# jhoobergs/Thesis-pbrt-v3

Hardware: AMD Instinct MI355X
Metric: Mrays/s (higher is better)
Workload: dtype f32; 1 GPU; Sponza-class atrium STAND-IN (311,728 tris, matte+plastic, point light; the reference ships no Sponza geometry) 700x700, halton 1024 spp, path maxdepth 5, bvh; spp_total=1024, tiles=16x16 round-robin over 1 GPU(s), parallelism=tile-dp1, film_merge=none (single GPU)

## Files before the change

thesis-pbrt-v3_amd/__init__.py:

```python
import ctypes as C
import os

import numpy as np

_HERE = os.path.dirname(os.path.abspath(__file__))
LIB_PATH = os.environ.get("HPRT_LIB") or os.path.join(_HERE, "lib", "libhprt.so")


class HprtError(RuntimeError):
    def __init__(self, code, msg):
        super().__init__("hprt error %d: %s" % (code, msg))
        self.code = code


E_INVALID, E_IO, E_PARSE, E_NO_DEVICE, E_DEVICE, E_UNSUPPORTED = -1, -2, -3, -4, -5, -6
RENDER_COUNT_WORK = 1
RENDER_PIXEL_STATS = 2
RENDER_COUNT_TRACED = 4
RENDER_TRACE_ALL = 8
RENDER_EXPORT_FOREIGN = 16
ACCEL_BVH, ACCEL_KDTREE, ACCEL_RBSP = 0, 1, 2
ACCEL_BSP = ACCEL_RBSP
KD_MAX_DEPTH = 64
RBSP_MAX_DEPTH = 64
# ... 181 lines not shown

class SceneDesc(C.Structure):
    _fields_ = [("nodes", C.c_void_p), ("n_nodes", C.c_uint32), ("prim_order", C.c_void_p), ("n_prims", C.c_uint32),
                ("shapes", C.POINTER(ShapeDesc)), ("n_shapes", C.c_uint32),
                ("materials", C.POINTER(MaterialDesc)), ("n_materials", C.c_uint32),
                ("lights", C.POINTER(LightDesc)), ("n_lights", C.c_uint32), ("light_strategy", C.c_int32),
                ("textures", C.c_void_p), ("n_textures", C.c_uint32),
                ("objects", C.c_void_p), ("n_objects", C.c_uint32), ("instances", C.c_void_p), ("n_instances", C.c_uint32),
                ("top", C.c_void_p), ("n_top", C.c_uint32)]


def _load():
    if not os.path.exists(LIB_PATH):
        raise ImportError("hprt: %s is missing — run `python thesis-pbrt-v3_amd/build.py` (hipcc, gfx950). "
                          "There is no CPU fallback." % LIB_PATH)
    lib = C.CDLL(LIB_PATH)
    vp, cp, i32, u32, u64, sz = C.c_void_p, C.c_char_p, C.c_int32, C.c_uint32, C.c_uint64, C.c_size_t
    P = C.POINTER
    sig = {
        "hprt_last_error": (cp, []),
        "hprt_version": (cp, []),
        "hprt_model_parse": (C.c_int, [cp, P(cp), C.c_int, P(vp)]),
        "hprt_model_load": (C.c_int, [cp, P(vp)]),
        "hprt_model_save": (C.c_int, [vp, cp]),
        "hprt_model_save_compact": (C.c_int, [vp, cp]),
        "hprt_model_destroy": (None, [vp]),
        "hprt_model_get_options": (C.c_int, [vp, P(RenderOptions)]),
        "hprt_model_set_options": (C.c_int, [vp, P(RenderOptions)]),
        "hprt_model_counts": (C.c_int, [vp, P(u64)]),
        "hprt_model_warnings": (cp, [vp]),
        "hprt_model_texture_info": (C.c_int, [vp, C.c_uint32, P(C.c_int32), P(C.c_float)]),
        "hprt_model_texture_level": (C.c_int, [vp, C.c_uint32, C.c_uint32, P(C.c_int32), vp]),
        "hprt_bvh_build": (C.c_int, [vp, P(vp)]),
        "hprt_bvh_build_from_bounds": (C.c_int, [sz, vp, vp, C.c_int, C.c_int, C.c_int, P(vp)]),
        "hprt_bvh_destroy": (None, [vp]),
        "hprt_bvh_info": (C.c_int, [vp, P(u32), P(C.c_float)]),
        "hprt_bvh_copy": (C.c_int, [vp, vp, vp]),
        "hprt_bvh_object_info": (C.c_int, [vp, C.c_uint32, P(u32), P(C.c_float)]),
        "hprt_bvh_object_copy": (C.c_int, [vp, C.c_uint32, vp, vp]),
        "hprt_bvhold_build": (C.c_int, [vp, vp, P(vp)]),
        "hprt_bvhold_build_from_bounds": (C.c_int, [sz, vp, vp, vp, P(vp)]),
        "hprt_bvhold_build_device": (C.c_int, [vp, vp, vp, vp, P(vp)]),
        "hprt_bvhold_build_device_from_bounds": (C.c_int, [sz, vp, vp, vp, vp, vp, P(vp)]),
        "hprt_scene_create": (C.c_int, [vp, C.c_int, P(vp)]),
        "hprt_scene_create_from_model": (C.c_int, [vp, vp, C.c_int, P(vp)]),
        "hprt_scene_destroy": (None, [vp]),
        "hprt_intersect": (C.c_int, [vp, sz, vp, vp, vp, vp, vp, vp, vp]),
        "hprt_occluded": (C.c_int, [vp, sz, vp, vp, vp, vp, vp]),
        "hprt_intersect_instanced": (C.c_int, [vp, sz, vp, vp, vp, vp, vp, vp, vp, vp]),
        "hprt_intersect_device": (C.c_int, [vp, sz, vp, vp, vp, vp, vp]),
        "hprt_occluded_device": (C.c_int, [vp, sz, vp, vp, vp]),
        "hprt_render": (C.c_int, [vp, P(RenderDesc), vp, vp, P(RenderStats)]),
        "hprt_film_resolve": (C.c_int, [vp, sz, C.c_float, vp]),
        "hprt_film_read": (C.c_int, [vp, vp, sz]),
        "hprt_pixel_stats_read": (C.c_int, [vp, vp, sz]),
        "hprt_write_pixel_stats": (C.c_int, [cp, vp, C.c_int, C.c_int]),
        "hprt_write_pfm": (C.c_int, [cp, vp, C.c_int, C.c_int]),
        "hprt_sample_radiance": (C.c_int, [vp, P(RenderOptions), sz, vp, vp, vp, vp]),
        "hprt_halton_permutations": (C.c_int, [vp, sz, P(sz)]),
        "hprt_comm_unique_id": (C.c_int, [vp]),
        "hprt_comm_create": (C.c_int, [vp, C.c_int, C.c_int, C.c_int, P(vp)]),
        "hprt_comm_info": (C.c_int, [vp, P(C.c_int), P(C.c_int), P(C.c_int)]),
        "hprt_comm_destroy": (None, [vp]),
        "hprt_film_gather": (C.c_int, [vp, vp, vp, sz, C.c_int, vp]),
        "hprt_film_gather_local": (C.c_int, [P(vp), P(vp), C.c_int, sz, C.c_int]),
        "hprt_film_gather_local_shutdown": (None, []),
        "hprt_scene_reserve": (C.c_int, [vp, P(RenderDesc)]),
        "hprt_film_records_read": (C.c_int, [vp, vp, sz, P(sz)]),
        "hprt_film_records_merge": (C.c_int, [vp, sz, vp, sz]),
        "hprt_model_accelerator": (C.c_int, [vp, vp, sz]),
        "hprt_kdtree_build": (C.c_int, [vp, P(vp)]),
        "hprt_kdtree_build_from_bounds": (C.c_int, [sz, vp, vp, C.c_int, C.c_int, C.c_float, C.c_int, C.c_int, P(vp)]),
        "hprt_kdtree_info": (C.c_int, [vp, P(u32)]),
        "hprt_kdtree_copy": (C.c_int, [vp, vp, vp]),
        "hprt_kdtree_destroy": (None, [vp]),
        "hprt_scene_attach_kdtree": (C.c_int, [vp, vp]),
        "hprt_kdinst_build": (C.c_int, [vp, P(vp)]),
        "hprt_kdinst_info": (C.c_int, [vp, P(u32)]),
        "hprt_kdinst_object_info": (C.c_int, [vp, u32, P(u32)]),
        "hprt_kdinst_copy": (C.c_int, [vp, vp, vp]),
        "hprt_kdinst_object_copy": (C.c_int, [vp, u32, vp, vp]),
        "hprt_kdinst_destroy": (None, [vp]),
        "hprt_scene_attach_kdinst": (C.c_int, [vp, vp]),
        "hprt_write_pixel_stats_accel": (C.c_int, [cp, vp, C.c_int, C.c_int, C.c_int]),
        "hprt_rbsp_build": (C.c_int, [vp, vp, P(vp)]),
        "hprt_rbsp_build_from_triangles": (C.c_int, [sz, vp, vp, P(vp)]),
        "hprt_rbsp_info": (C.c_int, [vp, P(u32)]),
        "hprt_rbsp_copy": (C.c_int, [vp, vp, vp, vp]),
        "hprt_rbsp_destroy": (None, [vp]),
        "hprt_scene_attach_rbsp": (C.c_int, [vp, vp]),
        "hprt_rbspkd_build": (C.c_int, [vp, vp, P(vp)]),
        "hprt_rbspkd_build_from_triangles": (C.c_int, [sz, vp, vp, P(vp)]),
        "hprt_rbspkd_info": (C.c_int, [vp, P(u32)]),
        "hprt_rbspkd_copy": (C.c_int, [vp, vp, vp, vp]),
        "hprt_rbspkd_destroy": (None, [vp]),
        "hprt_scene_attach_rbspkd": (C.c_int, [vp, vp]),
        "hprt_rbspinst_build": (C.c_int, [vp, vp, P(vp)]),
        "hprt_rbspkdinst_build": (C.c_int, [vp, vp, P(vp)]),
        "hprt_rbspinst_info": (C.c_int, [vp, P(u32)]),
        "hprt_rbspinst_object_info": (C.c_int, [vp, u32, P(u32)]),
        "hprt_rbspinst_copy": (C.c_int, [vp, vp, vp, vp]),
        "hprt_rbspinst_object_copy": (C.c_int, [vp, u32, vp, vp]),
        "hprt_rbspinst_destroy": (None, [vp]),
        "hprt_scene_attach_rbspinst": (C.c_int, [vp, vp]),
        "hprt_rbsp_build_device": (C.c_int, [vp, vp, vp, vp, P(vp)]),
        "hprt_rbsp_build_from_triangles_device": (C.c_int, [sz, vp, vp, vp, vp, P(vp)]),
        "hprt_rbspkd_build_device": (C.c_int, [vp, vp, vp, vp, P(vp)]),
        "hprt_rbspkd_build_from_triangles_device": (C.c_int, [sz, vp, vp, vp, vp, P(vp)]),
        "hprt_bsppaper_build_device": (C.c_int, [vp, vp, vp, vp, P(vp)]),
        "hprt_bsppaper_build_from_triangles_device": (C.c_int, [sz, vp, vp, vp, vp, P(vp)]),
        "hprt_bsppaperkd_build_device": (C.c_int, [vp, vp, vp, vp, P(vp)]),
        "hprt_bsppaperkd_build_from_triangles_device": (C.c_int, [sz, vp, vp, vp, vp, P(vp)]),
        "hprt_bsppaper_build": (C.c_int, [vp, vp, P(vp)]),
        "hprt_bsppaper_build_from_triangles": (C.c_int, [sz, vp, vp, P(vp)]),
        "hprt_bsppaper_info": (C.c_int, [vp, P(u32)]),
        "hprt_bsppaper_copy": (C.c_int, [vp, vp, vp]),
        "hprt_bsppaper_destroy": (None, [vp]),
        "hprt_scene_attach_bsppaper": (C.c_int, [vp, vp]),
        "hprt_bsppaperkd_build": (C.c_int, [vp, vp, P(vp)]),
        "hprt_bsppaperkd_build_from_triangles": (C.c_int, [sz, vp, vp, P(vp)]),
        "hprt_bsppaperkd_info": (C.c_int, [vp, P(u32)]),
        "hprt_bsppaperkd_copy": (C.c_int, [vp, vp, vp]),
        "hprt_bsppaperkd_destroy": (None, [vp]),
        "hprt_scene_attach_bsppaperkd": (C.c_int, [vp, vp]),
        "hprt_bsppaperinst_build": (C.c_int, [vp, vp, P(vp)]),
        "hprt_bsppaperkdinst_build": (C.c_int, [vp, vp, P(vp)]),
        "hprt_bsppaperinst_info": (C.c_int, [vp, P(u32)]),
        "hprt_bsppaperinst_object_info": (C.c_int, [vp, u32, P(u32)]),
        "hprt_bsppaperinst_copy": (C.c_int, [vp, vp, vp]),
        "hprt_bsppaperinst_object_copy": (C.c_int, [vp, u32, vp, vp]),
        "hprt_bsppaperinst_destroy": (None, [vp]),
        "hprt_scene_attach_bsppaperinst": (C.c_int, [vp, vp]),
        "hprt_bspnode_build": (C.c_int, [vp, vp, P(vp)]),
        "hprt_bspnode_build_from_triangles": (C.c_int, [sz, vp, vp, P(vp)]),
        "hprt_bspnodekd_build": (C.c_int, [vp, vp, P(vp)]),
        "hprt_bspnodekd_build_from_triangles": (C.c_int, [sz, vp, vp, P(vp)]),
        "hprt_bspnode_build_device": (C.c_int, [vp, vp, vp, vp, P(vp)]),
        "hprt_bspnode_build_from_triangles_device": (C.c_int, [sz, vp, vp, vp, vp, P(vp)]),
        "hprt_bspnodekd_build_device": (C.c_int, [vp, vp, vp, vp, P(vp)]),
        "hprt_bspnodekd_build_from_triangles_device": (C.c_int, [sz, vp, vp, vp, vp, P(vp)]),
        "hprt_scene_kd_counters": (C.c_int, [vp, vp]),
        "hprt_pixel_kd_stats_read": (C.c_int, [vp, vp, sz]),
        "hprt_write_pixel_stats_rbspkd": (C.c_int, [cp, vp, vp, C.c_int, C.c_int]),
    }
    debug = {}
    for prefix in ("kdinst", "rbspinst", "bsppaperinst"):
        debug["hprt_debug_%s_bounds" % prefix] = (C.c_int, [vp, C.c_int, vp])
        debug["hprt_debug_%s_set_tree" % prefix] = (C.c_int, [vp, C.c_int, sz, vp, sz, vp, vp])
    debug["hprt_debug_halton_index"] = (C.c_int, [P(RenderOptions), sz, vp, vp, vp, vp, vp, vp])
    debug["hprt_debug_shadow_grid"] = (C.c_int, [C.c_int])
    debug["hprt_debug_shadow_grid_info"] = (C.c_int, [vp, vp])
    debug["hprt_debug_shadow_grid_occluded"] = (C.c_int, [vp, sz, vp, vp, vp])
    debug["hprt_debug_shadow_grid_build"] = (C.c_int, [sz, vp, vp, C.c_uint32, vp, vp, sz, vp, sz])
    for name, (res, args) in list(sig.items()) + list(debug.items()):
        fn = getattr(lib, name)
        fn.restype = res
        fn.argtypes = args
    return lib, sorted(sig)


lib, EXPORTS = _load()


def _check(rc):
    if rc != 0:
        raise HprtError(rc, lib.hprt_last_error().decode("utf-8", "replace"))


def _ptr(a):
    return None if a is None else a.ctypes.data_as(C.c_void_p)


def version():
    return lib.hprt_version().decode()


_probe_lib = None


def _probe():
    global _probe_lib
    if _probe_lib is None:
        path = os.path.join(os.path.dirname(LIB_PATH), "libhprt_probe.so")
        if not os.path.exists(path):
            raise ImportError("hprt: %s is missing — run `python thesis-pbrt-v3_amd/build.py`" % path)
        p = C.CDLL(path)
        p.hprt_debug_device_halton.restype = C.c_int
        p.hprt_debug_device_halton.argtypes = [C.c_void_p, C.c_int, C.c_int, C.c_int, C.c_int, C.c_size_t, C.c_void_p, C.c_void_p, C.c_void_p]
        p.hprt_debug_device_bsdf.restype = C.c_int
        p.hprt_debug_device_bsdf.argtypes = [C.c_void_p, C.c_int, C.c_size_t] + [C.c_void_p] * 6
        _probe_lib = p
    return _probe_lib


SG_SINGLE, SG_PRIM_MASK = 0x80000000, 0x0fffffff


def debug_shadow_grid(on):
    return lib.hprt_debug_shadow_grid(int(on))


def shadow_grid_build(p9, light, res):
    p9 = np.ascontiguousarray(p9, np.float32).reshape(-1, 9)
    light = np.ascontiguousarray(light, np.float32)
    info = np.zeros(6, np.float64)
    _check(lib.hprt_debug_shadow_grid_build(p9.shape[0], _ptr(p9), _ptr(light), int(res), _ptr(info), None, 0, None, 0))
    R, n_entries = int(info[0]), int(info[1])
    cell_start = np.zeros(6 * R * R + 1, np.uint32); entries = np.zeros((max(1, n_entries), 2), np.uint32)
    _check(lib.hprt_debug_shadow_grid_build(p9.shape[0], _ptr(p9), _ptr(light), int(res), _ptr(info), _ptr(cell_start), cell_start.size, _ptr(entries), entries.shape[0]))
    entries = entries[:n_entries]
    return {"R": R, "eps": float(info[3]), "near": int(info[2]), "longest": int(info[4]), "seconds": float(info[5]), "cell_start": cell_start,
            "prim": (entries[:, 0] & SG_PRIM_MASK).astype(np.int64), "single": (entries[:, 0] & SG_SINGLE) != 0, "key": (entries[:, 1] & np.uint32(0xffff0000)).view(np.float32),
            "rect": np.stack([(entries[:, 1] >> s) & 15 for s in (0, 4, 8, 12)], axis=1).astype(np.int64)}


def debug_halton_index(opt, px, py, sample):
    px = np.ascontiguousarray(px, np.int32); py = np.ascontiguousarray(py, np.int32); sample = np.ascontiguousarray(sample, np.int64)
    a = np.zeros(px.shape[0], np.uint64); b = np.zeros(px.shape[0], np.uint64); bounds = np.zeros(4, np.int32)
    _check(lib.hprt_debug_halton_index(C.byref(opt), px.shape[0], _ptr(px), _ptr(py), _ptr(sample), _ptr(a), _ptr(b), _ptr(bounds)))
    return a, b, tuple(int(v) for v in bounds)


class Model:

    def __init__(self, handle):
        self._h = handle

    @staticmethod
    def parse(path, subst=None):
        kv = []
        for k, v in (subst or {}).items():
            kv += [k.encode(), v.encode()]
        arr = (C.c_char_p * max(1, len(kv)))(*kv)
        h = C.c_void_p()
        _check(lib.hprt_model_parse(path.encode(), arr, len(kv) // 2, C.byref(h)))
        return Model(h)

    @staticmethod
    def load(path):
        h = C.c_void_p()
        _check(lib.hprt_model_load(path.encode(), C.byref(h)))
        return Model(h)

    def save(self, path, compact=False):
        _check((lib.hprt_model_save_compact if compact else lib.hprt_model_save)(self._h, path.encode()))

    @property
    def options(self):
        o = RenderOptions()
        _check(lib.hprt_model_get_options(self._h, C.byref(o)))
        return o

    @options.setter
    def options(self, o):
        _check(lib.hprt_model_set_options(self._h, C.byref(o)))

    def counts(self):
        c = (C.c_uint64 * 7)()
        _check(lib.hprt_model_counts(self._h, c))
        return dict(zip(("shapes", "primitives", "triangles", "spheres", "materials", "lights", "textures"), [int(x) for x in c]))

    def texture(self, index):
        info = (C.c_int32 * 5)(); ma = C.c_float()
        _check(lib.hprt_model_texture_info(self._h, index, info, C.byref(ma)))
        levels = []
        for k in range(info[0]):
            wh = (C.c_int32 * 2)()
            _check(lib.hprt_model_texture_level(self._h, index, k, wh, None))
            a = np.zeros((wh[1], wh[0], 3), np.float32)
            _check(lib.hprt_model_texture_level(self._h, index, k, wh, _ptr(a)))
            levels.append(a)
        return {"levels": info[0], "trilinear": bool(info[1]), "wrap": info[2], "max_anisotropy": ma.value}, levels

    @property
    def accelerator(self):
        buf = C.create_string_buffer(256)
        _check(lib.hprt_model_accelerator(self._h, buf, 256))
        return buf.value.decode()

    def warnings(self):
        w = lib.hprt_model_warnings(self._h).decode()
        return [x for x in w.split("\n") if x]

    def __del__(self):
        if getattr(self, "_h", None) and lib is not None:
            lib.hprt_model_destroy(self._h)
            self._h = None


class Bvh:

    def __init__(self, model=None, handle=None):
        if handle is None:
            handle = C.c_void_p()
            _check(lib.hprt_bvh_build(model._h, C.byref(handle)))
        self._h = handle

    @staticmethod
    def from_bounds(bmin, bmax, max_node_prims=4, isect_cost=8, trav_cost=1):
        bmin = np.ascontiguousarray(bmin, np.float32); bmax = np.ascontiguousarray(bmax, np.float32)
        h = C.c_void_p()
        _check(lib.hprt_bvh_build_from_bounds(bmin.shape[0], _ptr(bmin), _ptr(bmax), max_node_prims, isect_cost, trav_cost, C.byref(h)))
        return Bvh(handle=h)

    def info(self):
        i = (C.c_uint32 * 4)()
        b = (C.c_float * 6)()
        _check(lib.hprt_bvh_info(self._h, i, b))
        return {"nodes": i[0], "prims": i[1], "leaves": i[2], "max_depth": i[3], "bounds": [float(x) for x in b]}

    def arrays(self):
        inf = self.info()
        nodes = np.zeros((inf["nodes"], 8), np.uint32)
        order = np.zeros(inf["prims"], np.uint32)
        _check(lib.hprt_bvh_copy(self._h, _ptr(nodes), _ptr(order)))
        return nodes, order

    def object_arrays(self, obj):
        i = (C.c_uint32 * 4)()
        _check(lib.hprt_bvh_object_info(self._h, obj, i, None))
        nodes = np.zeros((i[0], 8), np.uint32)
        order = np.zeros(i[1], np.uint32)
        _check(lib.hprt_bvh_object_copy(self._h, obj, _ptr(nodes), _ptr(order)))
        return nodes, order

    def __del__(self):
        if getattr(self, "_h", None) and lib is not None:
            lib.hprt_bvh_destroy(self._h)
            self._h = None


class BvhOldParams(C.Structure):
    _fields_ = [("split_method", C.c_int32), ("max_node_prims", C.c_int32)]


class BvhOldDeviceOpts(C.Structure):
    _fields_ = [("device", C.c_int), ("serial_treelet_max", C.c_uint32)]


class BvhOldDeviceStats(C.Structure):
    _fields_ = [("prims_sorted", C.c_uint64), ("sort_passes", C.c_uint64), ("treelets", C.c_uint64), ("treelets_host", C.c_uint64),
                ("launches", C.c_uint64), ("seconds_device", C.c_double)]

    def as_dict(self):
        return {n: getattr(self, n) for n, _ in self._fields_}


BVHOLD_SPLIT_METHODS = {"sah": 0, "hlbvh": 1, "middle": 2, "equal": 3}


class BvhOld(Bvh):

    def __init__(self, model=None, split_method=None, max_node_prims=None, device=None, serial_treelet_max=0, handle=None, build_stats=None):
        self.build_stats = build_stats
        if handle is None:
            handle, self.build_stats = BvhOld._build("build", (model._h,), split_method, max_node_prims, device, serial_treelet_max)
        self._h = handle

    @staticmethod
    def _build(how, head, split_method, max_node_prims, device, serial_treelet_max):
        prm = None
        if split_method is not None or max_node_prims is not None:
            sm = BVHOLD_SPLIT_METHODS[split_method] if isinstance(split_method, str) else (0 if split_method is None else int(split_method))
            prm = C.byref(BvhOldParams(sm, 4 if max_node_prims is None else int(max_node_prims)))
        h = C.c_void_p()
        if device is None:
            _check(getattr(lib, "hprt_bvhold_" + how)(*head, prm, C.byref(h)))
            return h, None
# ... 251 lines not shown
BSPNODE_CHOOSERS = ("arbitrary", "cluster", "random")
BSPNODE_FORMS = ("", "withkd", "fastkd")
BSPNODE_DEFAULT_SEED = 5489
BSPNODE_ACCELERATORS = tuple("bsp" + c + f for c in BSPNODE_CHOOSERS for f in BSPNODE_FORMS)


def _bspnode_params(accelerator, fastkd, n_directions, seed, isect_cost, trav_cost, kd_trav_cost, empty_bonus, max_prims, max_depth, threads):
    if accelerator not in BSPNODE_ACCELERATORS:
        raise ValueError("%r is no node-based BSP accelerator (%s)" % (accelerator, ", ".join(BSPNODE_ACCELERATORS)))
    k = BSPNODE_ACCELERATORS.index(accelerator)
    if (k % 3 == 2) != fastkd:
        raise ValueError("%r is built by %s" % (accelerator, "BspNode" if fastkd else "BspNodeKd"))
    return BspNodeParams(k // 3, k % 3, n_directions, seed, isect_cost, trav_cost, kd_trav_cost, empty_bonus, max_prims, max_depth, threads)


class BspNode(BspPaper):

    def __init__(self, model=None, accelerator=None, handle=None, n_directions=3, seed=BSPNODE_DEFAULT_SEED, isect_cost=80, trav_cost=5,
                 empty_bonus=0.0, max_prims=1, max_depth=-1, threads=0, device=None, min_candidates=0, max_edges=0, max_faces=0, max_face_edges=0, build_stats=None):
        self.build_stats = build_stats
        if handle is None:
            prm = None if accelerator is None else C.byref(_bspnode_params(accelerator, False, n_directions, seed, isect_cost, trav_cost, 1, empty_bonus,
                                                                          max_prims, max_depth, threads))
            handle, self.build_stats = _build_tree("bspnode", "build", (model._h,), prm,
                                                   _device_opts(BspBuildDeviceOpts, device, min_candidates, max_edges, max_faces, max_face_edges, 0))
        self._h = handle

    @staticmethod
    def from_triangles(p9, accelerator, n_directions=3, seed=BSPNODE_DEFAULT_SEED, isect_cost=80, trav_cost=5, empty_bonus=0.0, max_prims=1,
                       max_depth=-1, threads=0, device=None, min_candidates=0, max_edges=0, max_faces=0, max_face_edges=0):
        p9 = np.ascontiguousarray(p9, np.float32).reshape(-1, 9)
        prm = _bspnode_params(accelerator, False, n_directions, seed, isect_cost, trav_cost, 1, empty_bonus, max_prims, max_depth, threads)
        h, st = _build_tree("bspnode", "build_from_triangles", (p9.shape[0], _ptr(p9)), C.byref(prm),
                            _device_opts(BspBuildDeviceOpts, device, min_candidates, max_edges, max_faces, max_face_edges, 0))
        return BspNode(handle=h, build_stats=st)


class BspNodeKd(BspPaperKd):

    def __init__(self, model=None, accelerator=None, handle=None, n_directions=3, seed=BSPNODE_DEFAULT_SEED, isect_cost=80, trav_cost=5,
                 kd_trav_cost=1, empty_bonus=0.0, max_prims=1, max_depth=-1, threads=0, device=None, min_candidates=0, max_edges=0, max_faces=0, max_face_edges=0, build_stats=None):
        self.build_stats = build_stats
        if handle is None:
            prm = None if accelerator is None else C.byref(_bspnode_params(accelerator, True, n_directions, seed, isect_cost, trav_cost, kd_trav_cost,
                                                                          empty_bonus, max_prims, max_depth, threads))
            handle, self.build_stats = _build_tree("bspnodekd", "build", (model._h,), prm,
                                                   _device_opts(BspBuildDeviceOpts, device, min_candidates, max_edges, max_faces, max_face_edges, 0))
        self._h = handle

    @staticmethod
    def from_triangles(p9, accelerator, n_directions=3, seed=BSPNODE_DEFAULT_SEED, isect_cost=80, trav_cost=5, kd_trav_cost=1, empty_bonus=0.0,
                       max_prims=1, max_depth=-1, threads=0, device=None, min_candidates=0, max_edges=0, max_faces=0, max_face_edges=0):
        p9 = np.ascontiguousarray(p9, np.float32).reshape(-1, 9)
        prm = _bspnode_params(accelerator, True, n_directions, seed, isect_cost, trav_cost, kd_trav_cost, empty_bonus, max_prims, max_depth, threads)
        h, st = _build_tree("bspnodekd", "build_from_triangles", (p9.shape[0], _ptr(p9)), C.byref(prm),
                            _device_opts(BspBuildDeviceOpts, device, min_candidates, max_edges, max_faces, max_face_edges, 0))
        return BspNodeKd(handle=h, build_stats=st)


def bspnode_tree(model, accelerator=None, **kw):
    name = accelerator if accelerator is not None else model.accelerator
    fastkd = name.endswith("fastkd")
    if not fastkd:
        kw.pop("kd_trav_cost", None)
    return (BspNodeKd if fastkd else BspNode)(model, accelerator, **kw), ("attach_bsppaperkd" if fastkd else "attach_bsppaper")


class Scene:

    def __init__(self, model, bvh, device=-1):
        h = C.c_void_p()
        _check(lib.hprt_scene_create_from_model(model._h, bvh._h, device, C.byref(h)))
        self._h = h
        self._model = model

    @staticmethod
    def from_desc(desc, device=-1):
        h = C.c_void_p()
        _check(lib.hprt_scene_create(C.byref(desc), device, C.byref(h)))
        sc = Scene.__new__(Scene)
        sc._h = h
        sc._model = None
        return sc

    def attach_kdtree(self, kdtree):
        _check(lib.hprt_scene_attach_kdtree(self._h, kdtree._h))
        self._kdtree = kdtree

    def attach_kdinst(self, kdinst):
        _check(lib.hprt_scene_attach_kdinst(self._h, kdinst._h))
        self._kdinst = kdinst

    def attach_rbspinst(self, rbspinst):
        _check(lib.hprt_scene_attach_rbspinst(self._h, rbspinst._h))
        self._rbspinst = rbspinst

    def attach_bsppaperinst(self, bsppaperinst):
        _check(lib.hprt_scene_attach_bsppaperinst(self._h, bsppaperinst._h))
        self._bsppaperinst = bsppaperinst

    def attach_rbsp(self, rbsp):
        _check(lib.hprt_scene_attach_rbsp(self._h, rbsp._h))
        self._rbsp = rbsp

    def attach_rbspkd(self, rbspkd):
        _check(lib.hprt_scene_attach_rbspkd(self._h, rbspkd._h))
        self._rbspkd = rbspkd

    def attach_bsppaper(self, bsppaper):
        _check(lib.hprt_scene_attach_bsppaper(self._h, bsppaper._h))
        self._bsppaper = bsppaper

    def attach_bsppaperkd(self, bsppaperkd):
        _check(lib.hprt_scene_attach_bsppaperkd(self._h, bsppaperkd._h))
        self._bsppaperkd = bsppaperkd

    def kd_counters(self):
        out = np.zeros(2, np.uint64)
        _check(lib.hprt_scene_kd_counters(self._h, _ptr(out)))
        return int(out[0]), int(out[1])

    def intersect(self, o, d, tmax, count=False):
        o = np.ascontiguousarray(o, np.float32); d = np.ascontiguousarray(d, np.float32)
        tmax = np.ascontiguousarray(tmax, np.float32)
        n = tmax.shape[0]
        t = np.zeros(n, np.float32); prim = np.zeros(n, np.int32); bary = np.zeros((n, 3), np.float32)
        ctr = np.zeros(4, np.uint64) if count else None
        _check(lib.hprt_intersect(self._h, n, _ptr(o), _ptr(d), _ptr(tmax), _ptr(t), _ptr(prim), _ptr(bary), _ptr(ctr)))
        return (t, prim, bary, ctr) if count else (t, prim, bary)

    def intersect_instanced(self, o, d, tmax, count=False):
        o = np.ascontiguousarray(o, np.float32); d = np.ascontiguousarray(d, np.float32)
        tmax = np.ascontiguousarray(tmax, np.float32)
        n = tmax.shape[0]
        t = np.zeros(n, np.float32); prim = np.zeros(n, np.int32); inst = np.zeros(n, np.int32); bary = np.zeros((n, 3), np.float32)
        ctr = np.zeros(4, np.uint64) if count else None
        _check(lib.hprt_intersect_instanced(self._h, n, _ptr(o), _ptr(d), _ptr(tmax), _ptr(t), _ptr(prim), _ptr(inst), _ptr(bary), _ptr(ctr)))
        return (t, prim, inst, bary, ctr) if count else (t, prim, inst, bary)

    def occluded(self, o, d, tmax, count=False):
        o = np.ascontiguousarray(o, np.float32); d = np.ascontiguousarray(d, np.float32)
        tmax = np.ascontiguousarray(tmax, np.float32)
        n = tmax.shape[0]
        occ = np.zeros(n, np.uint8)
        ctr = np.zeros(4, np.uint64) if count else None
        _check(lib.hprt_occluded(self._h, n, _ptr(o), _ptr(d), _ptr(tmax), _ptr(occ), _ptr(ctr)))
        return (occ, ctr) if count else occ

    def shadow_grid_info(self):
        out = np.zeros(12, np.float64)
        _check(lib.hprt_debug_shadow_grid_info(self._h, _ptr(out)))
        return {"eligible": bool(out[0]), "R": int(out[1]), "entries": int(out[2]), "near": int(out[3]), "bytes": int(out[4]), "build_seconds": float(out[5]),
                "longest": int(out[6]), "mean": float(out[7]), "light": out[8:11].astype(np.float32), "render_launches": int(out[11])}

    def shadow_grid_occluded_device(self, n, rays7_ptr, occ_ptr):
        ms = C.c_float()
        _check(lib.hprt_debug_shadow_grid_occluded(self._h, n, rays7_ptr, occ_ptr, C.byref(ms)))
        return float(ms.value)

    def intersect_device(self, n, rays7_ptr, t_ptr, prim_ptr, bary_ptr=None, stream=None):
        _check(lib.hprt_intersect_device(self._h, n, rays7_ptr, t_ptr, prim_ptr, bary_ptr, stream))

    def occluded_device(self, n, rays7_ptr, occ_ptr, stream=None):
        _check(lib.hprt_occluded_device(self._h, n, rays7_ptr, occ_ptr, stream))

    def render(self, opt=None, tile_begin=0, tile_end=0, tile_stride=1, spp_chunk=0, count_work=False, film_ptr=None,
               stream=None, pixel_stats=False, count_traced=False, trace_all=False, export_foreign=False):
        opt = opt or self._model.options
        desc = RenderDesc()
        desc.opt = opt
        desc.tile_begin, desc.tile_end, desc.tile_stride = tile_begin, tile_end, tile_stride
        desc.spp_chunk = spp_chunk
        desc.flags = (RENDER_COUNT_WORK if count_work else 0) | (RENDER_PIXEL_STATS if pixel_stats else 0) | \
                     (RENDER_COUNT_TRACED if count_traced else 0) | (RENDER_TRACE_ALL if trace_all else 0) | \
                     (RENDER_EXPORT_FOREIGN if export_foreign else 0)
        self._film_shape = tuple(int(v) for v in (opt.film_bounds()[3] - opt.film_bounds()[1], opt.film_bounds()[2] - opt.film_bounds()[0]))
        st = RenderStats()
        _check(lib.hprt_render(self._h, C.byref(desc), film_ptr, stream, C.byref(st)))
        film = None
        if film_ptr is None:
            x0, y0, x1, y1 = opt.film_bounds()
            film = np.zeros((y1 - y0, x1 - x0, 4), np.float32)
            _check(lib.hprt_film_read(self._h, _ptr(film), film.shape[0] * film.shape[1]))
        return film, st.as_dict()

    def reserve(self, opt=None, tile_begin=0, tile_end=0, tile_stride=1, spp_chunk=0):
        desc = RenderDesc()
        desc.opt = opt or self._model.options
        desc.tile_begin, desc.tile_end, desc.tile_stride, desc.spp_chunk, desc.flags = tile_begin, tile_end, tile_stride, spp_chunk, 0
        _check(lib.hprt_scene_reserve(self._h, C.byref(desc)))

    def debug_poison(self, byte):
        lib.hprt_debug_poison_workspace.argtypes = [C.c_void_p, C.c_int]
        _check(lib.hprt_debug_poison_workspace(self._h, -1 if byte is None else int(byte)))

    def debug_device_halton(self, bounds_w, bounds_h, index, dim, sample_pixel_center=False, use_lds=False):
        index = np.ascontiguousarray(index, np.uint64); dim = np.ascontiguousarray(dim, np.int32)
        assert index.shape == dim.shape and index.ndim == 1
        out = np.zeros(index.shape[0], np.float32)
        _check(_probe().hprt_debug_device_halton(self._h, int(bounds_w), int(bounds_h), int(bool(sample_pixel_center)), int(bool(use_lds)),
                                                 index.shape[0], _ptr(index), _ptr(dim), _ptr(out)))
        return out

    def debug_device_bsdf(self, mode, shape, frame9, wo, wi, u):
        shape = np.ascontiguousarray(shape, np.int32)
        frame9 = np.ascontiguousarray(frame9, np.float32).reshape(-1, 9)
        wo = np.ascontiguousarray(wo, np.float32).reshape(-1, 3); wi = np.ascontiguousarray(wi, np.float32).reshape(-1, 3)
        u = np.ascontiguousarray(u, np.float32).reshape(-1, 2)
        n = shape.shape[0]
        assert shape.ndim == 1 and frame9.shape[0] == n and wo.shape[0] == n and wi.shape[0] == n and u.shape[0] == n
        out = np.zeros((n, 8), np.float32)
        _check(_probe().hprt_debug_device_bsdf(self._h, int(mode), n, _ptr(shape), _ptr(frame9), _ptr(wo), _ptr(wi), _ptr(u), _ptr(out)))
        return out

    def film_records(self):
        n = C.c_size_t()
        _check(lib.hprt_film_records_read(self._h, None, 0, C.byref(n)))
        out = np.zeros(n.value, FILM_RECORD)
        if n.value:
            _check(lib.hprt_film_records_read(self._h, _ptr(out), n.value, C.byref(n)))
        return out

    def pixel_stats(self):
        h, w = self._film_shape
        out = np.zeros((h, w, 7), np.uint64)
        _check(lib.hprt_pixel_stats_read(self._h, _ptr(out), h * w))
        return out

    def pixel_kd_stats(self):
        h, w = self._film_shape
        out = np.zeros((2, h, w), np.uint64)
        _check(lib.hprt_pixel_kd_stats_read(self._h, _ptr(out), h * w))
        return out

    def sample_radiance(self, px, py, sample, opt=None):
        opt = opt or self._model.options
        px = np.ascontiguousarray(px, np.int32); py = np.ascontiguousarray(py, np.int32)
        sample = np.ascontiguousarray(sample, np.int64)
        L = np.zeros((px.shape[0], 3), np.float32)
        _check(lib.hprt_sample_radiance(self._h, C.byref(opt), px.shape[0], _ptr(px), _ptr(py), _ptr(sample), _ptr(L)))
        return L

    def __del__(self):
        if getattr(self, "_h", None) and lib is not None:
            lib.hprt_scene_destroy(self._h)
            self._h = None


class Comm:

    @staticmethod
    def unique_id():
        buf = (C.c_uint8 * COMM_ID_BYTES)()
        _check(lib.hprt_comm_unique_id(buf))
        return bytes(buf)

    def __init__(self, unique_id, rank, n_ranks, device=-1):
        if len(unique_id) != COMM_ID_BYTES:
            raise ValueError("unique id must be %d bytes" % COMM_ID_BYTES)
        h = C.c_void_p()
        buf = (C.c_uint8 * COMM_ID_BYTES).from_buffer_copy(unique_id)
        _check(lib.hprt_comm_create(buf, rank, n_ranks, device, C.byref(h)))
        self._h = h

    def info(self):
        r, n, d = C.c_int(), C.c_int(), C.c_int()
        _check(lib.hprt_comm_info(self._h, C.byref(r), C.byref(n), C.byref(d)))
        return {"rank": r.value, "n_ranks": n.value, "device": d.value}

    def film_gather(self, scene, film_ptr, n_pixels, root=0, stream=None):
        _check(lib.hprt_film_gather(self._h, scene._h, film_ptr, n_pixels, root, stream))

    def __del__(self):
        if getattr(self, "_h", None) and lib is not None:
            lib.hprt_comm_destroy(self._h)
            self._h = None


def film_gather_local(scenes, film_ptrs, n_pixels, root=0):
    n = len(scenes)
    hs = (C.c_void_p * n)(*[s._h for s in scenes])
    fs = (C.c_void_p * n)(*[C.c_void_p(p) if p else None for p in (film_ptrs or [None] * n)])
    _check(lib.hprt_film_gather_local(hs, fs, n, n_pixels, root))


def film_records_merge(film_xyzw, records):
    assert film_xyzw.dtype == np.float32 and film_xyzw.flags.c_contiguous
    rec = np.ascontiguousarray(records, FILM_RECORD).copy()
    _check(lib.hprt_film_records_merge(_ptr(film_xyzw), film_xyzw.size // 4, _ptr(rec), rec.shape[0]))
    return film_xyzw


def film_resolve(film_xyzw, scale=1.0):
    f = np.ascontiguousarray(film_xyzw, np.float32)
    rgb = np.zeros(f.shape[:-1] + (3,), np.float32)
    _check(lib.hprt_film_resolve(_ptr(f), f.size // 4, C.c_float(scale), _ptr(rgb)))
    return rgb


def write_pixel_stats(prefix, stats7):
    stats7 = np.ascontiguousarray(stats7, np.uint64)
    _check(lib.hprt_write_pixel_stats(prefix.encode(), _ptr(stats7), stats7.shape[1], stats7.shape[0]))


def write_pixel_stats_accel(prefix, stats7, accel):
    stats7 = np.ascontiguousarray(stats7, np.uint64)
# ... 23 lines not shown
```

thesis-pbrt-v3_amd/csrc/capi_device.hip:

```cpp
#include <hip/hip_runtime.h>
#include <algorithm>
#include <cassert>
#include <chrono>
#include <cmath>
#include <cstring>
#include <functional>
#include <map>
#include <memory>
#include <string>
#include <vector>
#include "../../include/hprt.h"
#include "device/kernels.h"
#include "halton_tables.h"
#include "host_transform.h"
#include "hprt_internal.h"
#include "device_state.h"
#include "scene_layout.h"
#include "wide_bvh.h"

using namespace hprt;


namespace {

int CheckDevice(int device, int *chosen) {
    int n = 0;
    hipError_t e = hipGetDeviceCount(&n);
    if (e != hipSuccess || n <= 0) return SetError(HPRT_E_NO_DEVICE, "no HIP device available (hprt has no CPU fallback)");
    if (device < 0) { if (hipGetDevice(&device) != hipSuccess) device = 0; }
    if (device >= n) return SetError(HPRT_E_INVALID, "device ordinal out of range");
    if (hipSetDevice(device) != hipSuccess) return SetError(HPRT_E_DEVICE, "hipSetDevice failed");
    *chosen = device;
    return HPRT_OK;
}

struct PlaneAllocator {
    char *base; size_t off = 0, cap;
    template <typename T> T *take(size_t n) { off = (off + 255) & ~(size_t)255; T *p = (T *)(base + off); off += n * sizeof(T); return p; }
};
struct Workspace {
    PathStream path[2];
    HitStream hit;
    VertexStreams vs;
    float4 *pend[2];
    float4 *Lfinal;
};
const size_t kPlaneBytesPerSlot = 16 * (2 * 4 + 1 + 2 + 2 + 1 + 4 + 1) + 1, kInstancePlaneBytesPerSlot = 8 + 8;
size_t PlaneBytesPerSlot(bool instances) { return kPlaneBytesPerSlot + (instances ? kInstancePlaneBytesPerSlot : 0); }
size_t PlaneBytes(size_t n, bool instances) { return n * PlaneBytesPerSlot(instances) + 32 * 256; }

void CarvePlanes(char *base, size_t n, bool instances, Workspace *w) {
    PlaneAllocator a{base, 0, 0};
    auto rays = [&](RayStream &r) { r.a = a.take<float4>(n); r.b = a.take<float4>(n); };
    for (int k = 0; k < 2; ++k) { rays(w->path[k].ray); w->path[k].beta = a.take<float4>(n); w->path[k].L = a.take<float4>(n); }
    w->hit.a = a.take<float4>(n); w->hit.b = instances ? a.take<float2>(n) : nullptr;
    rays(w->vs.shadow); w->vs.occluded = a.take<uint8_t>(n);
    rays(w->vs.mis); w->vs.misHit.a = a.take<float4>(n); w->vs.misHit.b = instances ? a.take<float2>(n) : nullptr;
    w->vs.pendLight = a.take<float4>(n); w->vs.pendMis = a.take<float4>(n);
    for (int k = 0; k < 2; ++k) w->pend[k] = a.take<float4>(n);
    w->vs.pendBeta = w->pend[0]; w->vs.pendPrev = w->pend[1];
    w->Lfinal = a.take<float4>(n);
}

struct EventTimer {
    std::vector<hipEvent_t> pool; size_t used = 0;
    ~EventTimer() { for (hipEvent_t e : pool) (void)hipEventDestroy(e); }
    hipEvent_t get() {
        if (used == pool.size()) { hipEvent_t e; if (hipEventCreate(&e) != hipSuccess) return nullptr; pool.push_back(e); }
        return pool[used++];
    }
    void reset() { used = 0; }
};

void MakeCamera(const HprtRenderOptions &o, DevCamera *cam) {
    Xform camToScreen = xf_perspective(o.fov, 1e-2f, 1000.f);
    const float *sw = o.screen_window;
    Xform screenToRaster = xf_scale((float)o.xres, (float)o.yres, 1) * xf_scale(1 / (sw[1] - sw[0]), 1 / (sw[2] - sw[3]), 1) *
                           xf_translate(vec3(-sw[0], -sw[3], 0));
    Xform rasterToScreen = screenToRaster.inverse();
    Xform rasterToCamera = camToScreen.inverse() * rasterToScreen;
    cam->rasterToCamera = rasterToCamera.m;
    memcpy(cam->cameraToWorld.m, o.camera_to_world, 64);
    cam->lensRadius = o.lens_radius; cam->focalDistance = o.focal_distance;
    cam->dxCamera = xf_point(cam->rasterToCamera, vec3(1, 0, 0)) - xf_point(cam->rasterToCamera, vec3(0, 0, 0));
    cam->dyCamera = xf_point(cam->rasterToCamera, vec3(0, 1, 0)) - xf_point(cam->rasterToCamera, vec3(0, 0, 0));
}

int CheckDepth(int maxDepth) {
    if (5 + 8 * ((int64_t)maxDepth + 1) > 1000)
        return SetError(HPRT_E_UNSUPPORTED, "maxdepth above 123: a path could pass the 1,000 sampler dimensions of the reference's Halton tables");
    return HPRT_OK;
}

struct FrameSetup {
    FilmGeom fg; int ntx, nty; HaltonLayout hal; RenderParams rp;
    std::vector<uint32_t> pixelXY; std::vector<uint64_t> pixelOffset;
    std::vector<int32_t> localIndex;
    int W, H;
    uint64_t offX[128], offY[128];
};
int SetupFrame(const HprtRenderOptions &o, FrameSetup *f) {
    if (o.xres <= 0 || o.yres <= 0 || o.xres > 32768 || o.yres > 32768) return SetError(HPRT_E_INVALID, "film resolution out of range");
    if (o.filter_radius[0] != 0.5f || o.filter_radius[1] != 0.5f)
        return SetError(HPRT_E_UNSUPPORTED, "only the box filter with radius 0.5 is in the hot-path scope (SURVEY.md §2)");
    FilmGeom &fg = f->fg;
    fg.cx0 = (int)std::ceil(o.xres * o.crop[0]); fg.cx1 = (int)std::ceil(o.xres * o.crop[1]);
    fg.cy0 = (int)std::ceil(o.yres * o.crop[2]); fg.cy1 = (int)std::ceil(o.yres * o.crop[3]);
    fg.rx = o.filter_radius[0]; fg.ry = o.filter_radius[1];
    fg.sx0 = (int)std::floor((float)fg.cx0 + 0.5f - fg.rx); fg.sy0 = (int)std::floor((float)fg.cy0 + 0.5f - fg.ry);
    fg.sx1 = (int)std::ceil((float)fg.cx1 - 0.5f + fg.rx); fg.sy1 = (int)std::ceil((float)fg.cy1 - 0.5f + fg.ry);
    fg.maxSampleLuminance = o.max_sample_luminance;
    f->W = fg.cx1 - fg.cx0; f->H = fg.cy1 - fg.cy0;
    if (f->W <= 0 || f->H <= 0) return SetError(HPRT_E_INVALID, "empty crop window");
    f->ntx = (fg.sx1 - fg.sx0 + 15) / 16; f->nty = (fg.sy1 - fg.sy0 + 15) / 16;
    f->hal = MakeHaltonLayout(fg.sx1 - fg.sx0, fg.sy1 - fg.sy0);
    const uint64_t base = (uint64_t)HaltonPixelOffset(f->hal, 0, 0), stride = (uint64_t)std::max(1, f->hal.sampleStride);
    for (int m = 0; m < 128; ++m) {
        f->offX[m] = (uint64_t)HaltonPixelOffset(f->hal, m, 0);
        f->offY[m] = ((uint64_t)HaltonPixelOffset(f->hal, 0, m) + stride - base) % stride;
    }
    return HPRT_OK;
}
uint64_t TilePixelOffset(const FrameSetup &f, int x, int y) {
    const uint64_t stride = (uint64_t)std::max(1, f.hal.sampleStride);
    return f.hal.sampleStride > 1 ? (f.offX[((x % 128) + 128) % 128] + f.offY[((y % 128) + 128) % 128]) % stride : 0ull;
}
void AddTilePixels(FrameSetup *f, int tile) {
    const FilmGeom &fg = f->fg;
    int tx = tile % f->ntx, ty = tile / f->ntx;
    int x0 = fg.sx0 + tx * 16, x1 = std::min(x0 + 16, fg.sx1), y0 = fg.sy0 + ty * 16, y1 = std::min(y0 + 16, fg.sy1);
    for (int y = y0; y < y1; ++y)
        for (int x = x0; x < x1; ++x) {
            f->localIndex[(size_t)(y - fg.cy0) * f->W + (x - fg.cx0)] = (int32_t)f->pixelXY.size();
            f->pixelXY.push_back((uint32_t)x | ((uint32_t)y << 16));
            f->pixelOffset.push_back(TilePixelOffset(*f, x, y));
        }
}

}

extern "C" {

int hprt_scene_create(const HprtSceneDesc *d, int device, HprtScene **out) try {
    if (!d || !out) return SetError(HPRT_E_INVALID, "hprt_scene_create: null argument");
    SceneLayout L;
    if (int rc = BuildSceneLayout(*d, &L)) return rc;
    int dev;
    if (int rc = CheckDevice(device, &dev)) return rc;
    std::unique_ptr<HprtScene> sc(new HprtScene());
    sc->device = dev; sc->nPrims = L.nPrims;
    sc->topOrder = std::move(L.topOrder); sc->objectOrder = std::move(L.objectOrder); sc->objectPrimBase = std::move(L.objectPrimBase);
    sc->instanceObject = std::move(L.instanceObject); sc->instanced = L.instanced; sc->hasSubstrateBin = L.hasSubstrateBin;
    const std::vector<uint16_t> &perms = HaltonPermutations();
    std::vector<int32_t> primes(PrimeTable().begin(), PrimeTable().end()), primeSums(PrimeSumTable().begin(), PrimeSumTable().end());
    std::vector<uint64_t> magic(primes.size());
    for (size_t i = 0; i < primes.size(); ++i) magic[i] = 0xffffffffffffffffull / (uint64_t)primes[i] + 1ull;
    HIP_TRY(upload(sc->nodes, L.pairs)); HIP_TRY(upload(sc->tris, L.tris)); HIP_TRY(upload(sc->primVtx, L.primVtx));
    HIP_TRY(upload(sc->primN, L.primN)); HIP_TRY(upload(sc->vUV, L.vUV)); HIP_TRY(upload(sc->vS, L.vS));
    HIP_TRY(upload(sc->shapes, L.shapes)); HIP_TRY(upload(sc->materials, L.materials)); HIP_TRY(upload(sc->lights, L.lights));
    HIP_TRY(upload(sc->spheres, L.spheres)); HIP_TRY(upload(sc->instances, L.instances)); HIP_TRY(upload(sc->topEntry, L.topEntry));
    HIP_TRY(upload(sc->topEntryWide, L.topEntryWide)); HIP_TRY(upload(sc->lightFunc, L.lightFunc)); HIP_TRY(upload(sc->lightCdf, L.lightCdf));
    HIP_TRY(upload(sc->perms, perms)); HIP_TRY(upload(sc->primes, primes)); HIP_TRY(upload(sc->primeSums, primeSums));
    HIP_TRY(upload(sc->primeMagic, magic));
    HIP_TRY(upload(sc->textures, L.textures)); HIP_TRY(upload(sc->mipLevels, L.mipLevels)); HIP_TRY(upload(sc->texels, L.texels)); HIP_TRY(upload(sc->weightLut, L.weightLut));
    HIP_TRY(upload(sc->wide, L.wide)); HIP_TRY(upload(sc->leafBox, L.leafBox));
    HIP_TRY(upload(sc->envLights, L.envLights)); HIP_TRY(upload(sc->envData, L.envData));
    if (L.shadowGrid.eligible) {
        const ShadowGrid &sg = L.shadowGrid;
        static_assert(sizeof(SgEntry) == sizeof(uint2), "grid entries are read as 8-byte words");
        std::vector<SgEntry> padded(sg.entries);
        padded.push_back(SgEntry{0u, 0u});
        HIP_TRY(upload(sc->sgCells, sg.cellStart)); HIP_TRY(upload(sc->sgEntries, padded));
        sc->sg = DevShadowGrid{sc->sgCells.as<uint32_t>(), sc->sgEntries.as<uint2>(), (uint32_t)sg.entries.size(), sg.nNear, sg.R};
        sc->sgInfo.longest = sg.longest; sc->sgInfo.buildSeconds = sg.buildSeconds; sc->sgInfo.eps = sg.eps; sc->sgInfo.bytes = sg.bytes();
        for (int a = 0; a < 3; ++a) sc->sgInfo.light[a] = sg.light[a];
    }
    HIP_TRY(sc->counters.alloc(sizeof(DevCounters)));
    HIP_TRY(hipMemset(sc->counters.p, 0, sizeof(DevCounters)));
    HIP_TRY(sc->deepStack.alloc((size_t)HPRT_SPILL_STACK * HPRT_DEEP_THREADS * sizeof(uint2)));
    HIP_TRY(sc->workCounter.alloc(256));
    DevScene &dv = sc->dev;
    dv.pairs = sc->nodes.as<DevPair>(); dv.nPairs = (uint32_t)L.pairs.size();
    dv.wide = L.wide.empty() ? nullptr : sc->wide.as<DevWide>(); dv.nWide = (uint32_t)L.wide.size(); dv.leafBox = sc->leafBox.as<float4>();
    dv.tris = sc->tris.as<float4>(); dv.nPrims = L.nPrims;
    dv.primVtx = sc->primVtx.as<uint32_t>();
    dv.primN = sc->primN.as<float4>(); dv.vUV = sc->vUV.as<float>(); dv.vS = sc->vS.as<float>();
    dv.shapes = sc->shapes.as<DevShape>(); dv.nShapes = d->n_shapes;
    dv.materials = sc->materials.as<DevMaterial>();
    dv.lights = sc->lights.as<DevLight>(); dv.nLights = d->n_lights;
    dv.spheres = sc->spheres.as<DevSphere>(); dv.nSpheres = (uint32_t)L.spheres.size();
    dv.envLights = sc->envLights.as<DevEnvLight>(); dv.envData = sc->envData.as<float>(); dv.nEnvLights = (uint32_t)L.envLights.size();
    dv.textures = d->n_textures ? sc->textures.as<DevTexture>() : nullptr; dv.mipLevels = sc->mipLevels.as<DevMipLevel>();
    dv.texels = sc->texels.as<float>(); dv.weightLut = sc->weightLut.as<float>();
    dv.instances = sc->instances.as<DevInstance>(); dv.nInstances = d->n_instances;
    dv.topEntry = L.topEntry.empty() ? nullptr : sc->topEntry.as<float4>(); dv.nTopPrims = (uint32_t)L.topEntry.size();
    dv.topEntryWide = L.topEntryWide.empty() ? nullptr : sc->topEntryWide.as<float4>();
    dv.lightFunc = sc->lightFunc.as<float>(); dv.lightCdf = sc->lightCdf.as<float>(); dv.lightFuncInt = L.funcInt;
    dv.deepStack = sc->deepStack.as<uint2>();
    dv.perms = sc->perms.as<uint16_t>(); dv.primes = sc->primes.as<int32_t>(); dv.primeSums = sc->primeSums.as<int32_t>();
    dv.primeMagic = sc->primeMagic.as<uint64_t>();
    dv.worldRadius = L.worldRadius;
    dv.spatial = 0; dv.voxFunc = dv.voxCdf = dv.voxFuncInt = nullptr;
    dv.voxSlot = nullptr; dv.voxRequest = nullptr; dv.voxRequestCount = nullptr;
    for (int a = 0; a < 3; ++a) { dv.voxN[a] = L.voxN[a]; dv.wbMin[a] = L.wbMin[a]; dv.wbMax[a] = L.wbMax[a]; }
    if (L.lightStrategy == 2) {
        const uint64_t nVox = (uint64_t)dv.voxN[0] * (uint64_t)dv.voxN[1] * (uint64_t)dv.voxN[2];
        const uint64_t denseMaxFloats = [] { const char *e = getenv("HPRT_VOXEL_DENSE_MAX_MB"); return e ? (uint64_t)atoll(e) * (1ull << 18) : (1ull << 28); }();
        const uint64_t rowFloats = 2ull * d->n_lights + 2ull;
        const bool dense = nVox * rowFloats <= denseMaxFloats;
        uint64_t rows = nVox;
        if (!dense) {
            const uint64_t poolFloats = [] { const char *e = getenv("HPRT_VOXEL_POOL_MB"); return (e ? (uint64_t)atoll(e) : 4096ull) * (1ull << 18); }();
            rows = std::max<uint64_t>(1, std::min<uint64_t>(nVox, poolFloats / rowFloats));
        }
        HIP_TRY(sc->voxFunc.alloc(rows * d->n_lights * sizeof(float)));
        HIP_TRY(sc->voxCdf.alloc(rows * (d->n_lights + 1ull) * sizeof(float)));
        HIP_TRY(sc->voxFuncInt.alloc(rows * sizeof(float)));
        std::vector<float> ri(5 * 128);
        VoxelSamplePoints(ri.data());
        HIP_TRY(upload(sc->voxRi, ri));
        dv.spatial = 1;
        dv.voxFunc = sc->voxFunc.as<float>(); dv.voxCdf = sc->voxCdf.as<float>(); dv.voxFuncInt = sc->voxFuncInt.as<float>();
        sc->nVoxels = (uint32_t)nVox; sc->voxRows = (uint32_t)rows; sc->voxRowsUsed = 0;
        if (dense) LaunchVoxelDistributions(nullptr, dv, sc->voxRi.as<float>(), (uint32_t)nVox, sc->voxFunc.as<float>(), sc->voxCdf.as<float>(), sc->voxFuncInt.as<float>());
        else {
            HIP_TRY(sc->voxSlot.alloc(nVox * sizeof(int32_t)));
            HIP_TRY(hipMemset(sc->voxSlot.p, 0xff, nVox * sizeof(int32_t)));
            HIP_TRY(sc->voxRequest.alloc(nVox * sizeof(uint32_t)));
            HIP_TRY(sc->voxRequestCount.alloc(256));
            HIP_TRY(hipMemset(sc->voxRequestCount.p, 0, 256));
            dv.voxSlot = sc->voxSlot.as<int32_t>(); dv.voxRequest = sc->voxRequest.as<uint32_t>(); dv.voxRequestCount = sc->voxRequestCount.as<uint32_t>();
        }
        HIP_TRY(hipGetLastError());
        HIP_TRY(hipDeviceSynchronize());
    }
    HIP_TRY(hipHostMalloc((void **)&sc->hostCounts, (4096 + 256) * sizeof(uint32_t)));
    *out = sc.release();
    return HPRT_OK;
} catch (...) { return hprt::HandleException(); }

__attribute__((visibility("default"))) int hprt_debug_scene_walk(HprtScene *s) { return s && s->walk == HprtScene::Walk::Bvh && hprt::WideWalkInUse(s->dev) ? 1 : 0; }
__attribute__((visibility("default"))) int hprt_debug_shade_counts(HprtScene *s, int on, uint64_t *out2) {
    if (!s) return HPRT_E_INVALID;
    if (out2) { out2[0] = s->shadeDeferred; out2[1] = s->shadeRetried; }
    if (on && !s->shadeCountsOn) s->shadeDeferred = s->shadeRetried = s->shadeSpeculated = s->shadeRepaired = s->shadeFull = 0;
    s->shadeCountsOn = on != 0;
    return HPRT_OK;
}
__attribute__((visibility("default"))) int hprt_debug_speculated_counts(HprtScene *s, uint64_t *out3) {
    if (!s || !out3) return HPRT_E_INVALID;
    out3[0] = s->shadeSpeculated; out3[1] = s->shadeRepaired; out3[2] = s->shadeFull;
    return HPRT_OK;
}
static int g_speculateLight = -1;
static bool SpeculateLightEnabled() {
    static const bool fromEnv = [] { const char *e = getenv("HPRT_SPECULATE_LIGHT"); return !(e && atoi(e) == 0); }();
    return g_speculateLight < 0 ? fromEnv : g_speculateLight != 0;
}
__attribute__((visibility("default"))) int hprt_debug_speculate_light(int on) { const int was = SpeculateLightEnabled() ? 1 : 0; g_speculateLight = on; return was; }
static int g_foldRepair = -1;
static bool FoldRepairEnabled() {
    static const bool fromEnv = [] { const char *e = getenv("HPRT_FOLD_REPAIR"); return !(e && atoi(e) == 0); }();
    return g_foldRepair < 0 ? fromEnv : g_foldRepair != 0;
}
__attribute__((visibility("default"))) int hprt_debug_fold_repair(int on) { const int was = FoldRepairEnabled() ? 1 : 0; g_foldRepair = on; return was; }
__attribute__((visibility("default"))) int hprt_debug_poison_workspace(HprtScene *s, int byte) { if (!s) return HPRT_E_INVALID; s->poisonByte = byte < 0 ? -1 : (byte & 255); return HPRT_OK; }
__attribute__((visibility("default"))) int hprt_debug_capture_rays(HprtScene *s, int bounce, int kind, float *d_out7, size_t cap) {
    if (!s || kind < 0 || kind > 2 || cap > 0x7fffffffull) return HPRT_E_INVALID;
    s->capture.bounce = bounce; s->capture.kind = kind; s->capture.out7 = d_out7; s->capture.cap = cap; s->capture.n = 0;
    return HPRT_OK;
}
static int ApiStreams(HprtScene *s, size_t n, RayStream *rays, HitStream *hits);
static bool CountsKdShare(const HprtScene *s) {
    return s->walk == HprtScene::Walk::RbspKd || s->walk == HprtScene::Walk::BspPaperKd || s->walk == HprtScene::Walk::RbspKdInst ||
           s->walk == HprtScene::Walk::BspPaperKdInst;
}
static void Trace(HprtScene *s, hipStream_t st, bool anyHit, bool count, const uint32_t *queue, const uint32_t *countPtr, uint32_t countImm,
                  uint32_t gridItems, const RayStream &rays, const HitStream &hits, uint8_t *occ, DevCounters *counters, uint32_t *workCounter,
                  uint4 *rayStats = nullptr) {
    switch (s->walk) {
    case HprtScene::Walk::Kd: LaunchKdTrace(st, s->dev, s->kd, anyHit, count, queue, countPtr, countImm, gridItems, rays, hits, occ, counters, workCounter, rayStats); break;
    case HprtScene::Walk::Rbsp: LaunchRbspTrace(st, s->dev, s->rbsp, anyHit, count, queue, countPtr, countImm, gridItems, rays, hits, occ, counters, workCounter, rayStats); break;
    case HprtScene::Walk::RbspKd:
        LaunchRbspKdTrace(st, s->dev, DevRbspKd{s->rbsp, s->kdShare.as<unsigned long long>()}, anyHit, count, queue, countPtr, countImm, gridItems, rays,
                          hits, occ, counters, workCounter, rayStats);
        break;
    case HprtScene::Walk::BspPaper:
        LaunchBspPaperTrace(st, s->dev, s->bsppaper, anyHit, count, queue, countPtr, countImm, gridItems, rays, hits, occ, counters, workCounter, rayStats);
        break;
    case HprtScene::Walk::BspPaperKd:
        LaunchBspPaperKdTrace(st, s->dev, DevBspPaperKd{s->bsppaper, s->kdShare.as<unsigned long long>()}, anyHit, count, queue, countPtr, countImm,
                              gridItems, rays, hits, occ, counters, workCounter, rayStats);
        break;
    case HprtScene::Walk::KdInst:
        LaunchKdInstTrace(st, s->dev, s->kdinst, anyHit, count, queue, countPtr, countImm, gridItems, rays, hits, occ, counters, workCounter, rayStats);
        break;
    case HprtScene::Walk::RbspInst:
    case HprtScene::Walk::RbspKdInst:
        LaunchRbspInstTrace(st, s->dev, s->rbspinst, s->walk == HprtScene::Walk::RbspKdInst, anyHit, count, queue, countPtr, countImm, gridItems, rays, hits, occ,
                            counters, workCounter, rayStats);
        break;
    case HprtScene::Walk::BspPaperInst:
    case HprtScene::Walk::BspPaperKdInst:
        LaunchBspPaperInstTrace(st, s->dev, s->bsppaperinst, s->walk == HprtScene::Walk::BspPaperKdInst, anyHit, count, queue, countPtr, countImm, gridItems, rays,
                                hits, occ, counters, workCounter, rayStats);
        break;
    case HprtScene::Walk::Bvh: LaunchTrace(st, s->dev, anyHit, count, queue, countPtr, countImm, gridItems, rays, hits, occ, counters, workCounter, rayStats); break;
    }
}
static int g_shadowGrid = -1;
static bool ShadowGridInUse(const HprtScene *s) {
    return s->sg.entries != nullptr && g_shadowGrid != 0 && s->walk == HprtScene::Walk::Bvh && hprt::WideWalkInUse(s->dev) && !hprt::TraceProfileInUse();
}
__attribute__((visibility("default"))) int hprt_debug_shadow_grid(int on) { const int was = g_shadowGrid; g_shadowGrid = on; return was; }
__attribute__((visibility("default"))) int hprt_debug_shadow_grid_info(HprtScene *s, double out[12]) {
    if (!s || !out) return HPRT_E_INVALID;
    for (int a = 0; a < 3; ++a) out[8 + a] = s->sgInfo.light[a];
    out[11] = (double)s->sgInfo.renderLaunches;
    const bool has = s->sg.entries != nullptr;
    const double nCells = has ? 6.0 * s->sg.R * s->sg.R : 1.0;
    out[0] = has ? 1 : 0; out[1] = s->sg.R; out[2] = s->sg.nEntries; out[3] = s->sg.nNear; out[4] = (double)s->sgInfo.bytes;
    out[5] = s->sgInfo.buildSeconds; out[6] = s->sgInfo.longest; out[7] = has ? (s->sg.nEntries - s->sg.nNear) / nCells : 0.0;
    return HPRT_OK;
}
__attribute__((visibility("default"))) int hprt_debug_shadow_grid_occluded(HprtScene *s, size_t n, const float *d_rays7, uint8_t *d_occ, float *ms) try {
    if (!s || !d_rays7 || !d_occ || n == 0 || n > 0x7ffffff0ull) return SetError(HPRT_E_INVALID, "hprt_debug_shadow_grid_occluded: bad argument");
    if (!s->sg.entries) return SetError(HPRT_E_UNSUPPORTED, "hprt_debug_shadow_grid_occluded: the scene has no shadow grid");
    HIP_TRY(hipSetDevice(s->device));
    SceneCall call(s, nullptr);
    RayStream rays; HitStream hits;
    if (int rc = ApiStreams(s, n, &rays, &hits)) return rc;
    struct Events { hipEvent_t e[2] = {nullptr, nullptr}; ~Events() { for (auto x : e) if (x) (void)hipEventDestroy(x); } } ev;
    for (auto &x : ev.e) HIP_TRY(hipEventCreate(&x));
    LaunchPackRays(nullptr, d_rays7, (uint32_t)n, rays);
    HIP_TRY(hipEventRecord(ev.e[0], nullptr));
    LaunchShadowGrid(nullptr, s->dev, s->sg, nullptr, nullptr, (uint32_t)n, (uint32_t)n, rays, d_occ, s->workCounter.as<uint32_t>());
    HIP_TRY(hipEventRecord(ev.e[1], nullptr));
    HIP_TRY(hipGetLastError());
    HIP_TRY(hipDeviceSynchronize());
    if (ms) HIP_TRY(hipEventElapsedTime(ms, ev.e[0], ev.e[1]));
    return HPRT_OK;
} catch (...) { return hprt::HandleException(); }
__attribute__((visibility("default"))) int hprt_debug_trace_queued(HprtScene *s, size_t n, const float *d_rays7, const uint32_t *d_queue, int anyHit,
                                                                    float *d_scratch7, float ms[2]) try {
    if (!s || !d_rays7 || !d_queue || !d_scratch7 || !ms || n == 0 || n > 0x7ffffff0ull) return SetError(HPRT_E_INVALID, "hprt_debug_trace_queued: bad argument");
    HIP_TRY(hipSetDevice(s->device));
    SceneCall call(s, nullptr);
    RayStream rays; HitStream hits;
    if (int rc = ApiStreams(s, n, &rays, &hits)) return rc;
    DevBuf occ; HIP_TRY(occ.alloc(n));
    hipEvent_t e[3];
    for (auto &x : e) HIP_TRY(hipEventCreate(&x));
    LaunchPackRays(nullptr, d_rays7, (uint32_t)n, rays);
    HIP_TRY(hipEventRecord(e[0], nullptr));
    LaunchCaptureRays(nullptr, d_queue, (uint32_t)n, rays, d_scratch7, (uint32_t)n);
    HIP_TRY(hipEventRecord(e[1], nullptr));
    HitStream none; none.a = nullptr; none.b = nullptr;
    Trace(s, nullptr, anyHit != 0, false, d_queue, nullptr, (uint32_t)n, (uint32_t)n, rays, anyHit ? none : hits, anyHit ? occ.as<uint8_t>() : nullptr, nullptr, s->workCounter.as<uint32_t>());
    HIP_TRY(hipEventRecord(e[2], nullptr));
    HIP_TRY(hipDeviceSynchronize());
    HIP_TRY(hipEventElapsedTime(&ms[0], e[0], e[1])); HIP_TRY(hipEventElapsedTime(&ms[1], e[1], e[2]));
    for (auto &x : e) (void)hipEventDestroy(x);
    return HPRT_OK;
} catch (...) { return hprt::HandleException(); }
__attribute__((visibility("default"))) long long hprt_debug_captured(HprtScene *s) { return s ? (long long)s->capture.n : -1; }
__attribute__((visibility("default"))) int hprt_debug_stream_copy(int device, size_t bytes, int iters, double *best_gbs, double *mean_gbs) try {
    if (!best_gbs || !mean_gbs || iters < 1 || iters > 1000 || bytes < (1u << 20) || bytes > (64ull << 30)) return SetError(HPRT_E_INVALID, "hprt_debug_stream_copy: bad argument");
    int dev = 0;
    if (int rc = CheckDevice(device, &dev)) return rc;
    HIP_TRY(hipSetDevice(dev));
    DevBuf a, b;
    HIP_TRY(a.alloc(bytes)); HIP_TRY(b.alloc(bytes));
    HIP_TRY(hipMemset(a.p, 1, bytes)); HIP_TRY(hipMemset(b.p, 2, bytes));
    const size_t n = bytes / 16;
    hipEvent_t e0, e1;
    HIP_TRY(hipEventCreate(&e0)); HIP_TRY(hipEventCreate(&e1));
    LaunchStreamCopy(nullptr, a.as<float4>(), b.as<float4>(), n);
    HIP_TRY(hipDeviceSynchronize());
    double best = 0, sum = 0;
    for (int i = 0; i < iters; ++i) {
        HIP_TRY(hipEventRecord(e0, nullptr));
        LaunchStreamCopy(nullptr, a.as<float4>(), b.as<float4>(), n);
        HIP_TRY(hipEventRecord(e1, nullptr));
        HIP_TRY(hipEventSynchronize(e1));
        float ms = 0; HIP_TRY(hipEventElapsedTime(&ms, e0, e1));
        const double g = 2.0 * (double)(n * 16) / ((double)ms * 1e-3) / 1e9;
        best = std::max(best, g); sum += g;
    }
    (void)hipEventDestroy(e0); (void)hipEventDestroy(e1);
    *best_gbs = best; *mean_gbs = sum / iters;
    return HPRT_OK;
} catch (...) { return hprt::HandleException(); }
__attribute__((visibility("default"))) int hprt_debug_gather_probe(int device, int log2_records, int iters_per_lane, int launches, double *best_grecords_s, double *mean_grecords_s) try {
    if (!best_grecords_s || !mean_grecords_s || log2_records < 8 || log2_records > 26 || iters_per_lane < 1 || iters_per_lane > 100000 || launches < 1 || launches > 100)
        return SetError(HPRT_E_INVALID, "hprt_debug_gather_probe: bad argument");
    int dev = 0;
    if (int rc = CheckDevice(device, &dev)) return rc;
    HIP_TRY(hipSetDevice(dev));
    hipDeviceProp_t prop;
    HIP_TRY(hipGetDeviceProperties(&prop, dev));
    const uint32_t blocks = (uint32_t)prop.multiProcessorCount * 6u * 4u;
    DevBuf table, sink;
    const size_t bytes = (size_t)64 << log2_records;
    HIP_TRY(table.alloc(bytes)); HIP_TRY(sink.alloc(16));
    HIP_TRY(hipMemset(table.p, 0x5b, bytes));
    hipEvent_t e0, e1;
    HIP_TRY(hipEventCreate(&e0)); HIP_TRY(hipEventCreate(&e1));
    LaunchGatherProbe(nullptr, table.as<uint4>(), (uint32_t)log2_records, std::max(1, iters_per_lane / 10), blocks, sink.as<uint32_t>());
    HIP_TRY(hipDeviceSynchronize());
    double best = 0, sum = 0;
    for (int i = 0; i < launches; ++i) {
        HIP_TRY(hipEventRecord(e0, nullptr));
        LaunchGatherProbe(nullptr, table.as<uint4>(), (uint32_t)log2_records, iters_per_lane, blocks, sink.as<uint32_t>());
        HIP_TRY(hipEventRecord(e1, nullptr));
        HIP_TRY(hipEventSynchronize(e1));
        float ms = 0; HIP_TRY(hipEventElapsedTime(&ms, e0, e1));
        const double g = (double)blocks * 256.0 * (double)iters_per_lane / ((double)ms * 1e-3) / 1e9;
        best = std::max(best, g); sum += g;
    }
    (void)hipEventDestroy(e0); (void)hipEventDestroy(e1);
    *best_grecords_s = best; *mean_grecords_s = sum / launches;
    return HPRT_OK;
} catch (...) { return hprt::HandleException(); }

__global__ void k_debug_math(int fn, const float *x, const float *y, size_t n, double *o0, double *o1) {
    const size_t i = (size_t)blockIdx.x * blockDim.x + threadIdx.x;
    if (i >= n) return;
    double a = 0, b = 0;
    if (fn == 0) { float s, c; det_sincosf(x[i], &s, &c); a = (double)s; b = (double)c; }
    else if (fn == 1) a = (double)det_acosf(x[i]);
    else if (fn == 2) a = (double)det_atan2f(y[i], x[i]);
    else if (fn == 3) a = (double)det_logf(x[i]);
    else det_sincos_glibc_d((double)x[i], &a, &b);
    o0[i] = a; o1[i] = b;
}
__attribute__((visibility("default"))) int hprt_debug_device_math(int device, int fn, const float *x, const float *y, size_t n, double *out0, double *out1) try {
    if (fn < 0 || fn > 4 || !x || !y || !out0 || !out1 || n == 0 || n > ((size_t)1 << 28)) return SetError(HPRT_E_INVALID, "hprt_debug_device_math: bad argument");
    HIP_TRY(hipSetDevice(device));
    float *dx = nullptr, *dy = nullptr; double *d0 = nullptr, *d1 = nullptr;
    auto release = [&]() { (void)hipFree(dx); (void)hipFree(dy); (void)hipFree(d0); (void)hipFree(d1); };
    hipError_t e = hipMalloc((void **)&dx, n * 4);
    if (e == hipSuccess) e = hipMalloc((void **)&dy, n * 4);
    if (e == hipSuccess) e = hipMalloc((void **)&d0, n * 8);
    if (e == hipSuccess) e = hipMalloc((void **)&d1, n * 8);
    if (e == hipSuccess) e = hipMemcpy(dx, x, n * 4, hipMemcpyHostToDevice);
    if (e == hipSuccess) e = hipMemcpy(dy, y, n * 4, hipMemcpyHostToDevice);
    if (e == hipSuccess) {
        k_debug_math<<<dim3((unsigned)((n + 255) / 256)), dim3(256)>>>(fn, dx, dy, n, d0, d1);
        e = hipGetLastError();
    }
    if (e == hipSuccess) e = hipMemcpy(out0, d0, n * 8, hipMemcpyDeviceToHost);
    if (e == hipSuccess) e = hipMemcpy(out1, d1, n * 8, hipMemcpyDeviceToHost);
    release();
    if (e != hipSuccess) return SetError(HPRT_E_DEVICE, std::string("hprt_debug_device_math: ") + hipGetErrorString(e));
    return HPRT_OK;
} catch (...) { return hprt::HandleException(); }

struct TreeView {
    const char *what;
    const std::vector<BspNode> &nodes; const std::vector<uint32_t> &primIndices; uint32_t nPrims; const float *bounds;
    uint32_t M; const std::vector<float> *dirs; uint32_t todoMax;
    std::function<const char *(uint32_t *depth)> check;
    const std::vector<float> *axes = nullptr;
    uint32_t flagBits = 0, leafTag = 0;
};
static std::vector<uint32_t> InvertOrder(const std::vector<uint32_t> &order, uint32_t primBase) {
    std::vector<uint32_t> toOrdered(order.size());
    for (uint32_t i = 0; i < (uint32_t)order.size(); ++i) toOrdered[order[i]] = primBase + i;
    return toOrdered;
}
static uint32_t AppendTree(const std::vector<BspNode> &tree, const std::vector<uint32_t> &primIndices, const std::vector<uint32_t> &toOrdered,
                           uint32_t off, uint32_t mask, uint32_t leafTag, std::vector<uint2> *nodes, std::vector<uint32_t> *prims) {
    const uint32_t nodeBase = (uint32_t)nodes->size(), idxBase = (uint32_t)prims->size();
    for (const BspNode &nd : tree) {
        const uint32_t high = nd.b >> off;
        if ((nd.b & mask) != leafTag) nodes->push_back(make_uint2(nd.a, (nd.b & mask) | ((high + nodeBase) << off)));
        else nodes->push_back(make_uint2(high == 1u ? toOrdered[nd.a] : high == 0u ? nd.a : nd.a + idxBase, nd.b));
    }
    for (uint32_t p : primIndices) prims->push_back(toOrdered[p]);
    return nodeBase;
// ... 860 lines not shown
```

thesis-pbrt-v3_amd/csrc/capi_host.cpp:

```cpp
#include <algorithm>
#include <new>
#include <stdexcept>
#include <cmath>
#include <limits>
#include <vector>
#include <cstdio>
#include <cstring>
#include <map>
#include <memory>
#include <string>
#include <type_traits>
#include "../../include/hprt.h"
#include "bsp_cost_device.h"
#include "bspnode_cost_device.h"
#include "bspnode_builder.h"
#include "bvh_builder.h"
#include "halton_tables.h"
#include "hlbvh_build_device.h"
#include "hprt_internal.h"
#include "kdop_cost_device.h"
#include "scene_model.h"
#include "hprt_math.h"
#include "wide_bvh.h"
#include "shadow_grid.h"
// ... 1658 lines not shown
        o[0] *= scale; o[1] *= scale; o[2] *= scale;
    }
    return HPRT_OK;
} catch (...) { return hprt::HandleException(); }

int hprt_write_pixel_stats(const char *prefix, const uint64_t *stats7, int width, int height) try {
    return hprt_write_pixel_stats_accel(prefix, stats7, width, height, HPRT_ACCEL_BVH);
} catch (...) { return hprt::HandleException(); }
int hprt_write_pixel_stats_accel(const char *prefix, const uint64_t *stats7, int width, int height, int accel) try {
    if (!prefix || !stats7 || width <= 0 || height <= 0) return SetError(HPRT_E_INVALID, "hprt_write_pixel_stats: bad argument");
    if (accel != HPRT_ACCEL_BVH && accel != HPRT_ACCEL_KDTREE && accel != HPRT_ACCEL_RBSP) return SetError(HPRT_E_INVALID, "hprt_write_pixel_stats_accel: unknown accelerator");
    const int kd = accel == HPRT_ACCEL_KDTREE ? 5 : -1, kdP = accel == HPRT_ACCEL_KDTREE ? 6 : -1;
    const int bsp = accel == HPRT_ACCEL_RBSP ? 5 : -1, bspP = accel == HPRT_ACCEL_RBSP ? 6 : -1;
    const int field[8] = {1, 2, kd, kdP, bsp, bspP, 3, 4};
    return WriteStatMatrices(prefix, width, height, [&](int k, size_t i) { return field[k] < 0 ? 0ull : (unsigned long long)stats7[7 * i + field[k]]; });
} catch (...) { return hprt::HandleException(); }

int hprt_write_pixel_stats_rbspkd(const char *prefix, const uint64_t *stats7, const uint64_t *kd2, int width, int height) try {
    if (!prefix || !stats7 || !kd2 || width <= 0 || height <= 0) return SetError(HPRT_E_INVALID, "hprt_write_pixel_stats_rbspkd: bad argument");
    const size_t nPix = (size_t)width * (size_t)height;
    for (size_t i = 0; i < nPix; ++i)
        if (kd2[i] > stats7[7 * i + 5] || kd2[nPix + i] > stats7[7 * i + 6])
            return SetError(HPRT_E_INVALID, "hprt_write_pixel_stats_rbspkd: a pixel's kd share exceeds its interior-node count");
    const int field[8] = {1, 2, -1, -1, 5, 6, 3, 4}, kdPlane[8] = {-1, -1, 0, 1, 0, 1, -1, -1};
    return WriteStatMatrices(prefix, width, height, [&](int k, size_t i) {
        const unsigned long long kd = kdPlane[k] < 0 ? 0ull : (unsigned long long)kd2[(size_t)kdPlane[k] * nPix + i];
        return field[k] < 0 ? kd : (unsigned long long)stats7[7 * i + field[k]] - kd;
    });
} catch (...) { return hprt::HandleException(); }

int hprt_write_pfm(const char *path, const float *rgb, int width, int height) try {
    if (!path || !rgb || width <= 0 || height <= 0) return SetError(HPRT_E_INVALID, "hprt_write_pfm: bad argument");
    FILE *fp = fopen(path, "wb");
    if (!fp) return SetError(HPRT_E_IO, std::string("cannot create ") + path);
    bool ok = fprintf(fp, "PF\n%d %d\n-1.000000\n", width, height) > 0;
    for (int y = height - 1; y >= 0 && ok; --y) ok = fwrite(&rgb[3 * (size_t)y * width], sizeof(float), 3 * (size_t)width, fp) == 3 * (size_t)width;
    if (fclose(fp) != 0) ok = false;
    return ok ? HPRT_OK : SetError(HPRT_E_IO, std::string("write error on ") + path);
} catch (...) { return hprt::HandleException(); }

int hprt_film_records_merge(float *xyzw, size_t n_pixels, HprtFilmRecord *rec, size_t n) try {
    if (!xyzw || (n && !rec)) return SetError(HPRT_E_INVALID, "hprt_film_records_merge: null argument");
    std::sort(rec, rec + n, [](const HprtFilmRecord &a, const HprtFilmRecord &b) {
        return a.dest_pixel != b.dest_pixel ? a.dest_pixel < b.dest_pixel : a.src_tile < b.src_tile;
    });
    for (size_t i = 0; i < n; ++i) if (rec[i].dest_pixel >= n_pixels) return SetError(HPRT_E_INVALID, "film record outside the film");
    for (size_t i = 0; i < n; ++i) {
        float *px = xyzw + 4 * (size_t)rec[i].dest_pixel;
        px[0] += rec[i].xyz[0]; px[1] += rec[i].xyz[1]; px[2] += rec[i].xyz[2]; px[3] += rec[i].weight;
    }
    return HPRT_OK;
} catch (...) { return hprt::HandleException(); }

__attribute__((visibility("default"))) int hprt_debug_host_selftest(int failures[2]) try {
    if (!failures) return HPRT_E_INVALID;
    const float inf = std::numeric_limits<float>::infinity();
    int f = 0;
    if (!(next_up(-0.f) > 0.f)) ++f;
    if (!(next_down(0.f) < 0.f)) ++f;
    if (!(next_up(inf) == inf)) ++f;
    if (!(next_down(inf) < inf)) ++f;
    if (!(next_down(-inf) == -inf)) ++f;
    if (!(next_up(-inf) > -inf)) ++f;
    uint64_t state = 0x853c49e6748fea9bULL; const uint64_t inc = 0xda3e39cb94b95bdbULL;
    auto next32 = [&]() {
        uint64_t old = state;
        state = old * 0x5851f42d4c957f2dULL + inc;
        uint32_t xs = (uint32_t)(((old >> 18u) ^ old) >> 27u), rot = (uint32_t)(old >> 59u);
        return (xs >> rot) | (xs << ((~rot + 1u) & 31));
    };
    for (int i = 0; i < 100000; ++i) {
        float v;
        do { v = u2f(next32()); } while (std::isnan(v));
        if (std::isinf(v)) continue;
        if (std::nextafter(v, inf) != next_up(v)) ++f;
        if (std::nextafter(v, -inf) != next_down(v)) ++f;
    }
    failures[0] = f;
    f = 0;
    const float func[4] = {0, 1.f, 0.f, 3.f};
    float cdf[5], funcInt;
    dist1d_build(func, 4, cdf, &funcInt);
    float pdf;
    const float us[7] = {0.f, 0.125f, .24999f, .250001f, 0.625f, 0x1.fffffep-1f, 1.f};
    const int want[7] = {1, 1, 1, 3, 3, 3, 3};
    for (int k = 0; k < 7; ++k) {
        if (dist1d_sample_discrete(cdf, func, funcInt, 4, us[k], &pdf) != want[k]) ++f;
        if (pdf != (want[k] == 1 ? 0.25f : 0.75f)) ++f;
    }
    float u = .25f, uMax = .25f;
    for (int i = 0; i < 20; ++i) { u = next_down(u); uMax = next_up(uMax); }
    for (; u < uMax; u = next_up(u)) {
        int interval = dist1d_sample_discrete(cdf, func, funcInt, 4, u, &pdf);
        if (interval == 3) break;
        if (interval != 1) ++f;
    }
    if (!(u < uMax)) ++f;
    for (; u <= uMax; u = next_up(u))
        if (dist1d_sample_discrete(cdf, func, funcInt, 4, u, &pdf) != 3) ++f;
    failures[1] = f;
    return HPRT_OK;
} catch (...) { return hprt::HandleException(); }

__attribute__((visibility("default"))) int hprt_debug_wide_build(const void *nodes32, uint32_t n_nodes, void *out64, size_t cap, size_t *n_out, int *stack_need) try {
    if (!nodes32 || !n_out || !stack_need) return SetError(HPRT_E_INVALID, "hprt_debug_wide_build: null argument");
    const BvhNode *nd = (const BvhNode *)nodes32;
    const char *bad = CheckBvhNodes(nd, n_nodes, UINT32_MAX, nullptr);
    if (*bad) return SetError(HPRT_E_INVALID, std::string("hprt_debug_wide_build: ") + bad);
    std::vector<int32_t> leafRef(n_nodes, WIDE_NONE);
    for (uint32_t i = 0; i < n_nodes; ++i)
        if ((nd[i].countAxis & 3u) == 3u) leafRef[i] = (int32_t)(~(uint32_t)nd[i].offset & ~WIDE_LEAF_BOXED);
    std::vector<DevWide> wide;
    if (!BuildWide(nd, n_nodes, leafRef.data(), &wide, stack_need)) return SetError(HPRT_E_UNSUPPORTED, "the tree does not fit the four-wide grid");
    *n_out = wide.size();
    if (out64 && cap >= wide.size()) memcpy(out64, wide.data(), wide.size() * sizeof(DevWide));
    return HPRT_OK;
} catch (...) { return hprt::HandleException(); }

__attribute__((visibility("default"))) int hprt_debug_shape_inline(const HprtSceneDesc *d, uint32_t *tags, uint32_t *prim_shape, size_t prim_cap, size_t *n_prims,
                                                                    uint32_t *shape_flags, int32_t *shape_material, size_t shape_cap, size_t *n_shapes) try {
    if (!d || !n_prims || !n_shapes) return SetError(HPRT_E_INVALID, "hprt_debug_shape_inline: null argument");
    std::vector<uint32_t> t, ps, sf;
    std::vector<int32_t> smat;
    if (int rc = LayoutTagsForDebug(*d, &t, &ps, &sf, &smat)) return rc;
    *n_prims = t.size(); *n_shapes = sf.size();
    if (tags && prim_shape && prim_cap >= t.size()) { memcpy(tags, t.data(), 4 * t.size()); memcpy(prim_shape, ps.data(), 4 * ps.size()); }
    if (shape_flags && shape_material && shape_cap >= sf.size()) { memcpy(shape_flags, sf.data(), 4 * sf.size()); memcpy(shape_material, smat.data(), 4 * smat.size()); }
    return HPRT_OK;
} catch (...) { return hprt::HandleException(); }

__attribute__((visibility("default"))) int hprt_debug_shadow_grid_build(size_t n, const float *p9, const float light[3], uint32_t R, double info6[6],
                                                                         uint32_t *cell_start, size_t cell_cap, uint32_t *entries, size_t entry_cap) try {
    if (!n || !p9 || !light || !info6 || R == 0 || n >= (1u << 28)) return SetError(HPRT_E_INVALID, "hprt_debug_shadow_grid_build: bad argument");
    std::vector<float> tris(12 * n, 0.f);
    std::vector<uint8_t> single(n, 1);
    float lo[3] = {HPRT_INF, HPRT_INF, HPRT_INF}, hi[3] = {-HPRT_INF, -HPRT_INF, -HPRT_INF};
    for (size_t i = 0; i < n; ++i)
        for (int v = 0; v < 3; ++v)
            for (int a = 0; a < 3; ++a) {
                const float x = p9[9 * i + 3 * v + a];
                tris[12 * i + 4 * v + a] = x;
                if (x < lo[a]) lo[a] = x;
                if (x > hi[a]) hi[a] = x;
            }
    ShadowGrid g;
    BuildShadowGrid(tris.data(), single.data(), (uint32_t)n, light, lo, hi, R, (size_t)1 << 27, 0.0, &g);
    if (!g.eligible) return SetError(HPRT_E_UNSUPPORTED, "hprt_debug_shadow_grid_build: the lists do not fit");
    info6[0] = g.R; info6[1] = (double)g.entries.size(); info6[2] = g.nNear; info6[3] = g.eps; info6[4] = g.longest; info6[5] = g.buildSeconds;
    if (cell_start && cell_cap >= g.cellStart.size()) memcpy(cell_start, g.cellStart.data(), 4 * g.cellStart.size());
    if (entries && entry_cap >= g.entries.size()) memcpy(entries, g.entries.data(), 8 * g.entries.size());
    return HPRT_OK;
} catch (...) { return hprt::HandleException(); }

}
```

thesis-pbrt-v3_amd/csrc/device/shadow_grid.h:

```cpp
#pragma once
#include "kernels.h"

namespace hprt {

struct DevShadowGrid { const uint32_t *cellStart; const uint2 *entries; uint32_t nEntries, nNear, R; };

void LaunchShadowGrid(hipStream_t st, const DevScene &sc, const DevShadowGrid &g, const uint32_t *queue, const uint32_t *countPtr,
                      uint32_t countImm, uint32_t gridItems, const RayStream &rays, uint8_t *occ, uint32_t *workCounter);

}
```

thesis-pbrt-v3_amd/csrc/device/shadow_grid.hip:

```cpp
#include <hip/hip_runtime.h>
#include <algorithm>
#include <cstdlib>
#include "shadow_grid.h"
#include "dev_intersect.h"
#include "../shadow_grid.h"

namespace hprt {

typedef unsigned int u32x4 __attribute__((ext_vector_type(4)));
typedef unsigned int u32x2 __attribute__((ext_vector_type(2)));

#ifndef HPRT_SHADOW_GRID_WAVES
#define HPRT_SHADOW_GRID_WAVES 5
#endif

__device__ __forceinline__ uint32_t sg_cell(vec3 d, uint32_t R, float fineScale, uint32_t *sub) {
    const float x = -d.x, y = -d.y, z = -d.z;
    const float ax = fabsf(x), ay = fabsf(y), az = fabsf(z);
    const bool a0 = ax >= ay && ax >= az, a1 = !a0 && ay >= az;
    const float mj = a0 ? x : a1 ? y : z, a = a0 ? y : a1 ? z : x, b = a0 ? z : a1 ? x : y;
    const float m = fabsf(mj);
    const float u = a / m, v = b / m;
    int fu = (int)floorf((u + 1.f) * fineScale), fv = (int)floorf((v + 1.f) * fineScale);
    fu = sel_max(0, sel_min(16 * (int)R - 1, fu)); fv = sel_max(0, sel_min(16 * (int)R - 1, fv));
    const uint32_t face = (a0 ? 0u : a1 ? 2u : 4u) + (mj < 0 ? 1u : 0u);
    *sub = ((uint32_t)fu & 15u) | (((uint32_t)fv & 15u) << 4);
    return (face * R + ((uint32_t)fv >> 4)) * R + ((uint32_t)fu >> 4);
}
__device__ __forceinline__ bool sg_reaches(uint32_t w, uint32_t sub) {
    const uint32_t su = sub & 15u, sv = sub >> 4;
    return su >= (w & 15u) && su <= ((w >> 4) & 15u) && sv >= ((w >> 8) & 15u) && sv <= ((w >> 12) & 15u);
}

enum : int { SG_IDLE = 0, SG_RAY = 1, SG_HEAD = 2, SG_FIRST = 3, SG_TEST = 4, SG_BOX = 5 };

__global__ __launch_bounds__(HPRT_TRACE_BLOCK, HPRT_SHADOW_GRID_WAVES)
void k_shadow_grid(DevScene sc, DevShadowGrid g, const uint32_t *queue, const uint32_t *countPtr, uint32_t countImm, RayStream rays, uint8_t *occ,
                   uint32_t *workCounter, uint32_t chunk, uint32_t refillMin) {
    const uint32_t n = countPtr ? *countPtr : countImm;
    const uint32_t lane = __lane_id();
    const auto triRsrc = __builtin_amdgcn_make_buffer_rsrc((void *)sc.tris, 0, (int)(sc.nPrims * 48u), 0x00020000);
    const auto boxRsrc = __builtin_amdgcn_make_buffer_rsrc((void *)sc.leafBox, 0, (int)(sc.nPrims * 32u), 0x00020000);
    const auto entRsrc = __builtin_amdgcn_make_buffer_rsrc((void *)g.entries, 0, (int)((g.nEntries + 1u) * 8u), 0x00020000);
    const auto cellRsrc = __builtin_amdgcn_make_buffer_rsrc((void *)g.cellStart, 0, (int)((6u * g.R * g.R + 1u) * 4u), 0x00020000);
    const float robust = 1 + 2 * gamma_n(3);
    const float fineScale = 8.f * (float)g.R;
    int st = SG_IDLE;
    bool hit = false;
    uint32_t slot = 0u;
    uint32_t i = 0u, end = 0u, i2 = 0u, end2 = 0u;
    uint32_t ePrim = 0u;
    uint32_t sub = 0u;
    vec3 ro, invDir;
    float rayTMax = 0.f, lim = 0.f;
    RayShear shear; shear.k0 = shear.k1 = false; shear.Sx = shear.Sy = shear.Sz = 0.f;
    bool moreWork = n > 0;
    uint32_t localNext = 0u, localEnd = 0u;
    uint32_t window = 0u, windowBase = 0xffffffffu;
    while (true) {
        const unsigned long long idle = __ballot(st == SG_IDLE);
        if (moreWork && ((uint32_t)__popcll(idle) >= refillMin || idle == ~0ull)) {
            if (localNext >= localEnd) {
                uint32_t base = 0u;
                if (lane == 0) base = atomicAdd(workCounter, chunk);
                base = __builtin_amdgcn_readfirstlane(base);
                localNext = base < n ? base : n;
                localEnd = (base + chunk < n) ? base + chunk : n;
                if (localNext >= localEnd) moreWork = false;
                windowBase = 0xffffffffu;
            }
            const uint32_t want = (uint32_t)__popcll(idle);
            const uint32_t base = localNext;
            localNext = (localNext + want < localEnd) ? localNext + want : localEnd;
            const uint32_t rank = __builtin_amdgcn_mbcnt_hi((uint32_t)(idle >> 32), __builtin_amdgcn_mbcnt_lo((uint32_t)idle, 0u));
            uint32_t slotW = 0u;
            if (queue) {
                if (windowBase != base) { window = (base + lane < localEnd) ? queue[base + lane] : 0u; windowBase = base; }
                slotW = __shfl(window, (int)rank);
                window = (localNext + lane < localEnd) ? queue[localNext + lane] : 0u;
                windowBase = localNext;
            }
            if (st == SG_IDLE) {
                const uint32_t idx = base + rank;
                if (idx < localEnd) { slot = queue ? slotW : idx; hit = false; st = SG_RAY; }
            }
        }
        if (__ballot(st != SG_IDLE) == 0ull) {
            if (!moreWork) break;
            continue;
        }
        u32x4 r0 = {0u, 0u, 0u, 0u}, r1 = {0u, 0u, 0u, 0u}, r2 = {0u, 0u, 0u, 0u};
        u32x4 r3 = {0u, 0u, 0u, 0u};
        const uint32_t pi = ePrim & SG_PRIM_MASK;
        if (st == SG_TEST) {
            r0 = __builtin_amdgcn_raw_buffer_load_b128(triRsrc, pi * 48u, 0, 0);
            r1 = __builtin_amdgcn_raw_buffer_load_b128(triRsrc, pi * 48u + 16u, 0, 0);
            r2 = __builtin_amdgcn_raw_buffer_load_b128(triRsrc, pi * 48u + 32u, 0, 0);
            if (i + 1u < end) r3 = __builtin_amdgcn_raw_buffer_load_b128(entRsrc, (i + 1u) * 8u, 0, 0);
        } else if (st == SG_RAY) {
            r0 = __builtin_bit_cast(u32x4, rays.a[slot]);
            r1 = __builtin_bit_cast(u32x4, rays.b[slot]);
        } else if (st == SG_HEAD) {
            const u32x2 h = __builtin_amdgcn_raw_buffer_load_b64(cellRsrc, i * 4u, 0, 0);
            r3.x = h.x; r3.y = h.y;
        } else if (st == SG_FIRST) {
            r3 = __builtin_amdgcn_raw_buffer_load_b128(entRsrc, i * 8u, 0, 0);
        } else if (st == SG_BOX) {
            r0 = __builtin_amdgcn_raw_buffer_load_b128(boxRsrc, pi * 32u, 0, 0);
            r1 = __builtin_amdgcn_raw_buffer_load_b128(boxRsrc, pi * 32u + 16u, 0, 0);
        }
        asm volatile("" : "+v"(r0), "+v"(r1), "+v"(r2), "+v"(r3));
        auto leaf_reached = [&](float lx, float ly, float lz, float hx, float hy, float hz) -> bool {
            float tEn;
            return slab_test(lx, hx, ly, hy, lz, hz, ro, invDir, invDir.x < 0, invDir.y < 0, invDir.z < 0, robust, &tEn) && tEn < rayTMax;
        };
        bool done = false;
        bool haveNext = false;
        if (st == SG_RAY) {
            ro = vec3(__uint_as_float(r0.x), __uint_as_float(r0.y), __uint_as_float(r0.z));
            rayTMax = __uint_as_float(r0.w);
            const vec3 d(__uint_as_float(r1.x), __uint_as_float(r1.y), __uint_as_float(r1.z));
            invDir = vec3(1 / d.x, 1 / d.y, 1 / d.z);
            shear = ray_shear(d, invDir);
            const float dist2 = d.x * d.x + d.y * d.y + d.z * d.z;
            lim = rayTMax <= 1.f ? dist2 * (1.f + 0x1p-20f) : HPRT_INF;
            i = sg_cell(d, g.R, fineScale, &sub);
            st = SG_HEAD;
        } else if (st == SG_HEAD) {
            if (g.nNear != 0u) { i = 0u; end = g.nNear; i2 = r3.x; end2 = r3.y; }
            else { i = r3.x; end = r3.y; i2 = end2 = 0u; }
            st = SG_FIRST;
            if (i >= end) done = true;
        } else if (st == SG_FIRST) {
            haveNext = true;
        } else if (st == SG_TEST) {
            asm volatile("" : "+v"(r0), "+v"(r1), "+v"(r2));
            const vec3 p0(__uint_as_float(r0.x), __uint_as_float(r0.y), __uint_as_float(r0.z)), p1(__uint_as_float(r1.x), __uint_as_float(r1.y), __uint_as_float(r1.z)),
                       p2(__uint_as_float(r2.x), __uint_as_float(r2.y), __uint_as_float(r2.z));
            float b0, b1, b2, t;
            bool boxWanted = false;
            if (tri_test(p0, p1, p2, ro, rayTMax, shear, &b0, &b1, &b2, &t)) {
                if (ePrim & SG_SINGLE) {
                    if (leaf_reached(fminf(fminf(p0.x, p1.x), p2.x), fminf(fminf(p0.y, p1.y), p2.y), fminf(fminf(p0.z, p1.z), p2.z),
                                     fmaxf(fmaxf(p0.x, p1.x), p2.x), fmaxf(fmaxf(p0.y, p1.y), p2.y), fmaxf(fmaxf(p0.z, p1.z), p2.z))) { hit = true; done = true; }
                } else boxWanted = true;
            }
            if (boxWanted) st = SG_BOX;
            else if (!done) { ++i; haveNext = true; }
        } else if (st == SG_BOX) {
            if (leaf_reached(__uint_as_float(r0.x), __uint_as_float(r0.y), __uint_as_float(r0.z), __uint_as_float(r0.w), __uint_as_float(r1.x), __uint_as_float(r1.y))) { hit = true; done = true; }
            else { ++i; st = SG_FIRST; if (i >= end) { i = i2; end = end2; i2 = end2 = 0u; if (i >= end) done = true; } }
        }
        if (haveNext) {
            const bool in0 = i < end && !(__uint_as_float(r3.y & SG_KEY_MASK) > lim);
            const bool in1 = in0 && i + 1u < end && !(__uint_as_float(r3.w & SG_KEY_MASK) > lim);
            if (in0 && sg_reaches(r3.y, sub)) { ePrim = r3.x; st = SG_TEST; }
            else if (in1 && sg_reaches(r3.w, sub)) { ePrim = r3.z; ++i; st = SG_TEST; }
            else if (in1) { i += 2u; st = SG_FIRST; if (i >= end) { i = i2; end = end2; i2 = end2 = 0u; if (i >= end) done = true; } }
            else { i = i2; end = end2; i2 = end2 = 0u; st = SG_FIRST; if (i >= end) done = true; }
        }
        if (done) { occ[slot] = hit ? 1 : 0; st = SG_IDLE; }
    }
}

void LaunchShadowGrid(hipStream_t st, const DevScene &sc, const DevShadowGrid &g, const uint32_t *queue, const uint32_t *countPtr,
                      uint32_t countImm, uint32_t gridItems, const RayStream &rays, uint8_t *occ, uint32_t *workCounter) {
    if (gridItems == 0) return;
    (void)hipMemsetAsync(workCounter, 0, sizeof(uint32_t), st);
    static const uint32_t blockCap = [] { const char *e = getenv("HPRT_TRACE_MAX_BLOCKS"); return e ? (uint32_t)std::max(1, atoi(e)) : 0xffffffffu; }();
    static const uint32_t perCu = [] { const char *e = getenv("HPRT_SHADOW_GRID_PER_CU"); return e ? (uint32_t)std::min((int)HPRT_SHADOW_GRID_WAVES, std::max(1, atoi(e))) : (uint32_t)HPRT_SHADOW_GRID_WAVES; }();
    static const uint32_t chunkMax = [] { const char *e = getenv("HPRT_TRACE_CHUNK_MAX"); return e ? (uint32_t)atoi(e) : 512u; }();
    static const uint32_t refillMin = [] { const char *e = getenv("HPRT_SHADOW_GRID_REFILL"); return e ? (uint32_t)std::min(64, std::max(1, atoi(e))) : 32u; }();
    const uint32_t blocks = std::min((uint32_t)(((size_t)gridItems + HPRT_TRACE_BLOCK - 1) / HPRT_TRACE_BLOCK), std::min(256u * perCu, blockCap));
    const uint32_t nWaves = blocks * (HPRT_TRACE_BLOCK / 64);
    uint32_t chunk = gridItems / (nWaves * 4u);
    chunk = std::max(64u, std::min(chunkMax, chunk)) & ~63u;
    hipLaunchKernelGGL(k_shadow_grid, dim3(blocks), dim3(HPRT_TRACE_BLOCK), 0, st, sc, g, queue, countPtr, countImm, rays, occ, workCounter, chunk, refillMin);
}

}
```

thesis-pbrt-v3_amd/csrc/device_state.h:

```cpp
#pragma once
#include <hip/hip_runtime.h>
#include <algorithm>
#include <mutex>
#include <string>
#include <vector>
#include "../../include/hprt.h"
#include "device/kernels.h"
#include "device/kd_walk.h"
#include "device/rbsp_walk.h"
#include "device/rbspkd_walk.h"
#include "device/bsppaper_walk.h"
#include "device/bsppaperkd_walk.h"
#include "device/kdinst_walk.h"
#include "device/rbspinst_walk.h"
#include "device/bsppaperinst_walk.h"
#include "device/shadow_grid.h"
#include "hprt_internal.h"

#define HIP_TRY(expr)                                                                                   \
    do {                                                                                                \
        hipError_t e__ = (expr);                                                                        \
        if (e__ != hipSuccess)                                                                          \
            return hprt::SetError(HPRT_E_DEVICE, std::string(#expr) + ": " + hipGetErrorString(e__));   \
    } while (0)

namespace hprt {

struct DevBuf {
    void *p = nullptr; size_t bytes = 0;
    ~DevBuf() { if (p) (void)hipFree(p); }
    hipError_t alloc(size_t n) {
        if (p && bytes >= n) return hipSuccess;
        if (p) { (void)hipFree(p); p = nullptr; bytes = 0; }
        if (n == 0) return hipSuccess;
        hipError_t e = hipMalloc(&p, n);
        if (e == hipSuccess) bytes = n;
        return e;
    }
    template <typename T> T *as() const { return (T *)p; }
};
template <typename T> hipError_t upload(DevBuf &b, const std::vector<T> &v) {
    hipError_t e = b.alloc(std::max<size_t>(v.size() * sizeof(T), 16));
    if (e != hipSuccess || v.empty()) return e;
    return hipMemcpy(b.p, v.data(), v.size() * sizeof(T), hipMemcpyHostToDevice);
}

}

struct HprtScene;
namespace hprt {
struct SceneCall {
    std::unique_lock<std::mutex> lk; HprtScene *s; hipStream_t st;
    SceneCall(HprtScene *scene, hipStream_t stream);
    void leave_async();
};
}

struct HprtScene {
    int device = 0;
    std::mutex mu;
    hipEvent_t lastUse = nullptr; bool lastUsePending = false;
    hprt::DevScene dev;
    hprt::DevBuf textures, mipLevels, texels, weightLut;
    hprt::DevBuf nodes, tris, primVtx, primN, vUV, vS, shapes, materials, lights, spheres, instances, topEntry, topEntryWide, lightFunc, lightCdf, perms, primes, primeSums, primeMagic;
    hprt::DevBuf envLights, envData;
    hprt::DevBuf wide, leafBox;
    hprt::DevBuf sgCells, sgEntries; hprt::DevShadowGrid sg{};
    struct ShadowGridInfo { uint32_t longest = 0; double buildSeconds = 0, eps = 0; size_t bytes = 0; float light[3] = {0, 0, 0}; uint64_t renderLaunches = 0; } sgInfo;
    hprt::DevBuf counters, workCounter, deepStack;
    struct Capture { int bounce = -1, kind = 0; float *out7 = nullptr; size_t cap = 0, n = 0; } capture;
    bool shadeCountsOn = false; uint64_t shadeDeferred = 0, shadeRetried = 0;
    uint64_t shadeSpeculated = 0, shadeRepaired = 0, shadeFull = 0;
    int poisonByte = -1;
    hprt::DevBuf voxFunc, voxCdf, voxFuncInt, voxRi;
    hprt::DevBuf voxSlot, voxRequest, voxRequestCount, retryQueues;
    uint32_t voxRows = 0, voxRowsUsed = 0, nVoxels = 0;
    hprt::DevBuf rayStats, pixelStatsLocal, pixelStatsFilm; bool pixelStatsValid = false;
    hprt::DevBuf planes;
    hprt::DevBuf apiRays, apiHits;
    hprt::DevBuf queues, queueCounts;
    hprt::DevBuf pixelXY, pixelOffset, Lall, film, irregular, irregularCount;
    hprt::DevBuf exOwnBegin, exOwnSrc, exOwnSample, exOwnPre, exFDest, exFDestBegin, exFGroupBegin, exFSrc, exFSample;
    hprt::DevBuf foreignRecords, exGroupDest, exGroupTile; uint32_t nForeignRecords = 0; bool foreignExported = false;
    int filmW = 0, filmH = 0;
    float *lastFilm = nullptr;
    uint32_t *hostCounts = nullptr;
    size_t filmPixels = 0;
    uint32_t nPrims = 0;
    enum class Walk { Bvh, Kd, Rbsp, RbspKd, BspPaper, BspPaperKd, KdInst, RbspInst, RbspKdInst, BspPaperInst, BspPaperKdInst } walk = Walk::Bvh;
    hprt::DevBuf treeNodes, treePrims, treeAxes; hprt::DevKd kd{}; hprt::DevRbsp rbsp{}; hprt::DevBspPaper bsppaper{};
    hprt::DevBuf kdShare, pixelKdLocal, pixelKdFilm; bool pixelKdValid = false;
    std::vector<uint32_t> topOrder; bool instanced = false;
    bool hasSubstrateBin = false;
    hprt::DevBuf instEntries; hprt::DevKdInst kdinst{}; hprt::DevRbspInst rbspinst{}; hprt::DevBspPaperInst bsppaperinst{};
    std::vector<std::vector<uint32_t>> objectOrder; std::vector<uint32_t> objectPrimBase; std::vector<int32_t> instanceObject;
    ~HprtScene() { if (hostCounts) (void)hipHostFree(hostCounts); if (lastUse) (void)hipEventDestroy(lastUse); }
};

inline hprt::SceneCall::SceneCall(HprtScene *scene, hipStream_t stream) : lk(scene->mu), s(scene), st(stream) {
    if (s->lastUsePending && s->lastUse) (void)hipStreamWaitEvent(st, s->lastUse, 0);
}
inline void hprt::SceneCall::leave_async() {
    if (!s->lastUse && hipEventCreateWithFlags(&s->lastUse, hipEventDisableTiming) != hipSuccess) { s->lastUse = nullptr; (void)hipStreamSynchronize(st); s->lastUsePending = false; return; }
    s->lastUsePending = hipEventRecord(s->lastUse, st) == hipSuccess;
    if (!s->lastUsePending) (void)hipStreamSynchronize(st);
}
```

thesis-pbrt-v3_amd/csrc/scene_layout.cpp:

```cpp
#include <algorithm>
#include <cmath>
#include <cstdlib>
#include <cstring>
#include <utility>
#include "scene_layout.h"
#include "bvh_builder.h"
#include "device/dev_intersect.h"
#include "hprt_internal.h"
#include "wide_bvh.h"

namespace hprt {
namespace {

float RoughnessToAlpha(float roughness) {
    roughness = sel_max(roughness, (float)1e-3);
    float x = std::log(roughness);
    return 1.62142f + 0.819955f * x + 0.1734f * x * x + 0.0171201f * x * x * x + 0.000640711f * x * x * x * x;
}

bool TriangleIsBogus(vec3 p0, vec3 p1, vec3 p2, const float *uv0, const float *uv1, const float *uv2) {
    float u0x = 0, u0y = 0, u1x = 1, u1y = 0, u2x = 1, u2y = 1;
    if (uv0) { u0x = uv0[0]; u0y = uv0[1]; u1x = uv1[0]; u1y = uv1[1]; u2x = uv2[0]; u2y = uv2[1]; }
    float duv02x = u0x - u2x, duv02y = u0y - u2y, duv12x = u1x - u2x, duv12y = u1y - u2y;
    vec3 dp02 = p0 - p2, dp12 = p1 - p2;
// ... 359 lines not shown
        if (L.envData.size() + nFloats > 0x7fffffffull) return SetError(HPRT_E_UNSUPPORTED, "infinite light maps too large");
        L.envData.resize(L.envData.size() + nFloats);
        float *condFunc = L.envData.data() + e.off, *condCdf = condFunc + (size_t)height * width, *condInt = condCdf + (size_t)height * (width + 1),
              *margCdf = condInt + height;
        const float fwidth = 0.5f / std::min(width, height);
        for (int v = 0; v < height; ++v) {
            const float vp = (v + .5f) / (float)height;
            const float sinTheta = det_sinf(HPRT_PI * (v + .5f) / height);
            for (int u = 0; u < width; ++u) {
                const float up = (u + .5f) / (float)width;
                float y = luminance(HostMipLookupWidth(tx, up, vp, fwidth));
                y *= sinTheta;
                condFunc[(size_t)v * width + u] = y;
            }
            dist1d_build(condFunc + (size_t)v * width, width, condCdf + (size_t)v * (width + 1), &condInt[v]);
        }
        dist1d_build(condInt, height, margCdf, &e.margFuncInt);
        DevLight &o = L.lights[l];
        o.type = 4; o.shape = (int32_t)L.envLights.size();
        L.envLights.push_back(e);
    }
    return HPRT_OK;
}

int LayoutLightDistribution(Work &w) {
    const HprtSceneDesc *d = &w.d;
    SceneLayout &L = w.L;
    vec3 wbLo, wbHi;
    if (d->n_nodes) {
        const BvhNode &root = ((const BvhNode *)d->nodes)[0];
        wbLo = vec3(root.bmin[0], root.bmin[1], root.bmin[2]); wbHi = vec3(root.bmax[0], root.bmax[1], root.bmax[2]);
        vec3 c = div_by(wbLo + wbHi, 2.f);
        bool inside = c.x >= wbLo.x && c.x <= wbHi.x && c.y >= wbLo.y && c.y <= wbHi.y && c.z >= wbLo.z && c.z <= wbHi.z;
        L.worldRadius = inside ? dist(c, wbHi) : 0.f;
    }
    for (int a = 0; a < 3; ++a) { L.wbMin[a] = wbLo.get(a); L.wbMax[a] = wbHi.get(a); }
    L.lightFunc.assign(std::max<uint32_t>(1, d->n_lights), 1.f); L.lightCdf.assign(d->n_lights + 1, 0.f);
    if (L.lightStrategy == 1)
        for (uint32_t l = 0; l < d->n_lights; ++l) {
            const HprtLightDesc &in = d->lights[l];
            const rgb I(in.I[0], in.I[1], in.I[2]);
            rgb power;
            if (in.type == 0) power = I * (4 * HPRT_PI);
            else if (in.type == 1) power = I * HPRT_PI * L.worldRadius * L.worldRadius;
            else if (in.type == 3) power = HPRT_PI * L.worldRadius * L.worldRadius * HostMipLookupWidth(d->textures[in.texture], .5f, .5f, .5f);
            else {
                const HprtShapeDesc &ls = d->shapes[in.shape];
                float area;
                if (ls.kind == 1) area = ls.phi_max * ls.radius * (ls.z_max - ls.z_min);
                else {
                    const int32_t *v = &ls.indices[3 * (size_t)((int32_t)l - ls.area_light)];
                    const vec3 p0(ls.P[3 * v[0]], ls.P[3 * v[0] + 1], ls.P[3 * v[0] + 2]), p1(ls.P[3 * v[1]], ls.P[3 * v[1] + 1], ls.P[3 * v[1] + 2]),
                               p2(ls.P[3 * v[2]], ls.P[3 * v[2] + 1], ls.P[3 * v[2] + 2]);
                    area = (float)(0.5 * (double)length(cross(p1 - p0, p2 - p0)));
                }
                power = I * (float)(in.two_sided ? 2 : 1) * area * HPRT_PI;
            }
            L.lightFunc[l] = luminance(power);
        }
    if (d->n_lights) dist1d_build(L.lightFunc.data(), (int)d->n_lights, L.lightCdf.data(), &L.funcInt);
    if (L.lightStrategy == 2) {
        const vec3 diag = wbHi - wbLo;
        const int me = (diag.x > diag.y && diag.x > diag.z) ? 0 : (diag.y > diag.z ? 1 : 2);
        const float bmax = diag.get(me);
        for (int a = 0; a < 3; ++a) L.voxN[a] = std::max(1, int(std::round(diag.get(a) / bmax * 64)));
    }
    return HPRT_OK;
}

int LayoutPairs(Work &w) {
    SceneLayout &L = w.L;
    L.pairs.resize((size_t)w.pairBase[w.aggs.size()]);
    for (size_t ai = 0; ai < w.aggs.size(); ++ai) {
        const Agg &g = w.aggs[ai];
        if (g.nNodes == 0) continue;
        const BvhNode *nd = g.nodes;
        std::vector<int32_t> ref(g.nNodes);
        int32_t nextPair = (int32_t)w.pairBase[ai] + 1;
        for (uint32_t i = 0; i < g.nNodes; ++i) {
            if ((nd[i].countAxis & 3u) == 3u) {
                ref[i] = ~(int32_t)(w.primBase[ai] + (uint32_t)nd[i].offset);
                const size_t last = (size_t)w.primBase[ai] + (uint32_t)nd[i].offset + (nd[i].countAxis >> 2) - 1u;
                L.tris[3 * last].w = u2f(f2u(L.tris[3 * last].w) | TAG_LAST);
            } else ref[i] = nextPair++;
        }
        auto fill = [&](DevPair &p, uint32_t c0, uint32_t c1, uint32_t meta) {
            const BvhNode &a = nd[c0], &b = nd[c1];
            p.x[0] = a.bmin[0]; p.x[1] = b.bmin[0]; p.x[2] = a.bmax[0]; p.x[3] = b.bmax[0];
            p.y[0] = a.bmin[1]; p.y[1] = b.bmin[1]; p.y[2] = a.bmax[1]; p.y[3] = b.bmax[1];
            p.z[0] = a.bmin[2]; p.z[1] = b.bmin[2]; p.z[2] = a.bmax[2]; p.z[3] = b.bmax[2];
            p.ref0 = ref[c0]; p.ref1 = ref[c1]; p.meta = meta; p.pad = 0u;
        };
        fill(L.pairs[w.pairBase[ai]], 0u, 0u, PAIR_SINGLE);
        for (uint32_t i = 0; i < g.nNodes; ++i) {
            if ((nd[i].countAxis & 3u) == 3u) continue;
            fill(L.pairs[(size_t)ref[i]], i + 1u, (uint32_t)nd[i].offset, nd[i].countAxis & 3u);
        }
    }
    return HPRT_OK;
}

int LayoutWide(Work &w) {
    SceneLayout &L = w.L;
    w.wideBase.assign(w.aggs.size(), -1);
    bool wideOk = L.nPrims < (1u << 28);
    int wideNeedTop = 0, wideNeedObject = 0;
    for (size_t ai = 0; ai < w.aggs.size() && wideOk; ++ai) {
        const Agg &g = w.aggs[ai];
        if (g.nNodes == 0) continue;
        const BvhNode *nd = g.nodes;
        std::vector<int32_t> leafRefW(g.nNodes, WIDE_NONE);
        if (L.leafBox.empty()) { L.leafBox.assign(2 * (size_t)L.nPrims, make_float4(0.f, 0.f, 0.f, 0.f)); L.primSingle.assign(L.nPrims, 0); }
        for (uint32_t i = 0; i < g.nNodes; ++i) {
            if ((nd[i].countAxis & 3u) != 3u) continue;
            const uint32_t firstPrim = w.primBase[ai] + (uint32_t)nd[i].offset, count = nd[i].countAxis >> 2;
            bool single = count == 1u && (f2u(L.tris[3 * (size_t)firstPrim].w) & TAG_KIND_MASK) == 0u;
            if (single) {
                const float4 *v = &L.tris[3 * (size_t)firstPrim];
                const float c[3][3] = {{v[0].x, v[1].x, v[2].x}, {v[0].y, v[1].y, v[2].y}, {v[0].z, v[1].z, v[2].z}};
                for (int a = 0; a < 3 && single; ++a) {
                    bool posZero = false, negZero = false;
                    for (int k = 0; k < 3; ++k) { if (c[a][k] != c[a][k]) single = false; if (c[a][k] == 0.f) { if (f2u(c[a][k]) >> 31) negZero = true; else posZero = true; } }
                    const float mn = std::min(std::min(c[a][0], c[a][1]), c[a][2]), mx = std::max(std::max(c[a][0], c[a][1]), c[a][2]);
                    if ((posZero && negZero) || f2u(mn) != f2u(nd[i].bmin[a]) || f2u(mx) != f2u(nd[i].bmax[a])) single = false;
                }
            }
            uint32_t r = ~firstPrim;
            if (!single) r &= ~WIDE_LEAF_BOXED;
            else L.primSingle[firstPrim] = 1;
            leafRefW[i] = (int32_t)r;
            for (uint32_t k = 0; k < count; ++k) {
                L.leafBox[2 * (size_t)(firstPrim + k)] = make_float4(nd[i].bmin[0], nd[i].bmin[1], nd[i].bmin[2], nd[i].bmax[0]);
                L.leafBox[2 * (size_t)(firstPrim + k) + 1] = make_float4(nd[i].bmax[1], nd[i].bmax[2], 0.f, 0.f);
            }
        }
        int need = 0;
        w.wideBase[ai] = (int32_t)L.wide.size();
        if (!BuildWide(nd, g.nNodes, leafRefW.data(), &L.wide, &need)) wideOk = false;
        if (ai == 0) wideNeedTop = need; else wideNeedObject = std::max(wideNeedObject, need);
    }
    if (!wideOk || wideNeedTop + (w.d.n_instances ? 1 + wideNeedObject : 0) > HPRT_WIDE_STACK_MAX || w.wideBase[0] != 0) { L.wide.clear(); L.leafBox.clear(); L.primSingle.clear(); }
    return HPRT_OK;
}

int LayoutShadowGrid(Work &w) {
    SceneLayout &L = w.L;
    const int mode = ShadowGridModeFromEnv();
    if (mode == 0 || w.d.n_lights != 1 || L.lights.size() != 1 || L.lights[0].type != 0 || w.d.n_instances != 0 || w.d.n_objects != 0 ||
        !L.spheres.empty() || L.wide.empty() || L.nPrims == 0 || L.nPrims >= (1u << 28))
        return HPRT_OK;
    for (uint32_t i = 0; i < L.nPrims; ++i) if ((f2u(L.tris[3 * (size_t)i].w) & TAG_KIND_MASK) != 0u) return HPRT_OK;
    static_assert(sizeof(float4) == 16, "triangle records are read as 12 floats per primitive");
    const size_t capMb = [] { const char *e = getenv("HPRT_SHADOW_GRID_MAX_MB"); return e ? (size_t)std::max(1l, atol(e)) : (size_t)1024; }();
    BuildShadowGrid(&L.tris[0].x, L.primSingle.data(), L.nPrims, L.lights[0].pos, L.wbMin, L.wbMax, ShadowGridResFromEnv(), capMb * ((1u << 20) / sizeof(SgEntry)), mode < 0 ? SG_MAX_CANDIDATES : 0.0, &L.shadowGrid);
    return HPRT_OK;
}

int LayoutInstances(Work &w) {
    const HprtSceneDesc *d = &w.d;
    SceneLayout &L = w.L;
    L.instances.resize(d->n_instances);
    for (uint32_t i = 0; i < d->n_instances; ++i) {
        const HprtInstanceDesc &in = d->instances[i];
        DevInstance &o = L.instances[i];
        memcpy(o.i2w.m, in.instance_to_world, 64); memcpy(o.w2i.m, in.world_to_instance, 64);
        const size_t ai = 1 + (size_t)in.object;
        o.root = w.aggs[ai].nPrims > 1 ? (int32_t)w.pairBase[ai] : ~(int32_t)w.primBase[ai];
        bool ident = true;
        for (int r = 0; r < 4; ++r) for (int c = 0; c < 4; ++c) if (o.i2w.m[r][c] != (r == c ? 1.f : 0.f)) ident = false;
        o.identity = ident ? 1u : 0u; o.pad[0] = o.pad[1] = 0u;
        if (!L.wide.empty()) o.pad[0] = w.aggs[ai].nPrims > 1 ? (uint32_t)w.wideBase[ai] : ((~(uint32_t)w.primBase[ai]) & ~WIDE_LEAF_FIRST);
    }
    if (!d->n_instances) return HPRT_OK;
    const uint32_t nTop = w.aggs[0].nPrims;
    L.topEntry.assign(nTop, make_float4(0.f, 0.f, 0.f, 0.f));
    if (!L.wide.empty()) L.topEntryWide.assign(nTop, make_float4(0.f, 0.f, 0.f, 0.f));
    for (uint32_t oi = 0; oi < nTop; ++oi) {
        float4 *r = &L.tris[3 * ((size_t)w.primBase[0] + oi)];
        const uint32_t tag = f2u(r[0].w);
        if ((tag & TAG_KIND_MASK) != TAG_INSTANCE) continue;
        const DevInstance &in = L.instances[f2u(r[2].w)];
        const float (*m)[4] = in.w2i.m;
        if (!(m[3][0] == 0.f && m[3][1] == 0.f && m[3][2] == 0.f && m[3][3] == 1.f)) continue;
        r[0] = make_float4(m[0][0], m[0][1], m[0][2], u2f(tag | TAG_INST_INLINE));
        r[1] = make_float4(m[1][0], m[1][1], m[1][2], r[1].w);
        r[2] = make_float4(m[2][0], m[2][1], m[2][2], r[2].w);
        L.topEntry[oi] = make_float4(m[0][3], m[1][3], m[2][3], u2f((uint32_t)in.root));
        if (!L.wide.empty()) L.topEntryWide[oi] = make_float4(m[0][3], m[1][3], m[2][3], u2f(in.pad[0]));
    }
    return HPRT_OK;
}

}

int BuildSceneLayout(const HprtSceneDesc &d, SceneLayout *out) {
    Work w{d, *out};
    w.inlineMaterialMax = TAG_MATERIAL_MAX;
    if (const char *e = getenv("HPRT_INLINE_MATERIAL_MAX")) { const long v = atol(e); w.inlineMaterialMax = v < 0 ? 0u : (uint32_t)std::min<long>(v, (long)TAG_MATERIAL_MAX); }
    for (int (*stage)(Work &) : {ValidateArrays, ValidateShapes, GatherAggregates, CheckAggregates, ValidateLights}) if (int rc = stage(w)) return rc;
    out->nPrims = w.primBase.back();
    out->topOrder.assign(d.prim_order, d.prim_order + d.n_prims);
    out->instanced = d.n_instances != 0;
    for (uint32_t k = 0; k < d.n_objects; ++k) {
        out->objectOrder.emplace_back(d.objects[k].prim_order, d.objects[k].prim_order + d.objects[k].n_prims);
        out->objectPrimBase.push_back(w.primBase[1 + (size_t)k]);
    }
    for (uint32_t i = 0; i < d.n_instances; ++i) out->instanceObject.push_back(d.instances[i].object);
    for (int (*stage)(Work &) : {LayoutShapes, LayoutPrimitives, LayoutMaterials, LayoutTextures, LayoutLights, LayoutEnvLights,
                                 LayoutLightDistribution, LayoutPairs, LayoutWide, LayoutInstances, LayoutShadowGrid})
        if (int rc = stage(w)) return rc;
    return HPRT_OK;
}

int LayoutTagsForDebug(const HprtSceneDesc &d, std::vector<uint32_t> *tags, std::vector<uint32_t> *primShape, std::vector<uint32_t> *shapeFlags,
                       std::vector<int32_t> *shapeMaterial) {
    SceneLayout L;
    if (int rc = BuildSceneLayout(d, &L)) return rc;
    for (uint32_t i = 0; i < L.nPrims; ++i) { tags->push_back(f2u(L.tris[3 * (size_t)i].w)); primShape->push_back(f2u(L.tris[3 * (size_t)i + 1].w)); }
    for (const DevShape &s : L.shapes) { shapeFlags->push_back(s.flags); shapeMaterial->push_back(s.material); }
    return HPRT_OK;
}

void VoxelSamplePoints(float *out) {
    const int bases[5] = {2, 3, 5, 7, 11};
    for (int b = 0; b < 5; ++b)
        for (uint32_t i = 0; i < 128; ++i) {
            float v;
            if (b == 0) {
                uint32_t n = i;
                n = (n << 16) | (n >> 16); n = ((n & 0x00ff00ffu) << 8) | ((n & 0xff00ff00u) >> 8); n = ((n & 0x0f0f0f0fu) << 4) | ((n & 0xf0f0f0f0u) >> 4);
                n = ((n & 0x33333333u) << 2) | ((n & 0xccccccccu) >> 2); n = ((n & 0x55555555u) << 1) | ((n & 0xaaaaaaaau) >> 1);
                v = (float)((double)n * 0x1p-32);
            } else {
                const int base = bases[b];
                const float invBase = (float)1 / (float)base;
                uint64_t reversedDigits = 0, a = i;
                float invBaseN = 1;
                while (a) { uint64_t next = a / base, digit = a - next * base; reversedDigits = reversedDigits * base + digit; invBaseN *= invBase; a = next; }
                v = sel_min((float)reversedDigits * invBaseN, HPRT_ONE_MINUS_EPS);
            }
            out[128 * b + i] = v;
        }
}

}

extern "C" __attribute__((visibility("default"))) int hprt_debug_voxel_points(float out[640]) { if (!out) return HPRT_E_INVALID; hprt::VoxelSamplePoints(out); return HPRT_OK; }
```

thesis-pbrt-v3_amd/csrc/scene_layout.h:

```cpp
#pragma once
#include <cstdint>
#include <vector>
#include "../../include/hprt.h"
#include "device/dev_scene.h"
#include "shadow_grid.h"

namespace hprt {

struct SceneLayout {
    std::vector<DevPair> pairs;
    std::vector<DevWide> wide;
    std::vector<float4> leafBox, tris, primN;
    std::vector<uint32_t> primVtx;
    std::vector<float> vUV, vS;
    std::vector<DevShape> shapes;
    std::vector<DevSphere> spheres;
    std::vector<DevMaterial> materials;
    std::vector<DevTexture> textures;
    std::vector<DevMipLevel> mipLevels;
    std::vector<float> texels, weightLut;
    std::vector<DevLight> lights;
    std::vector<DevEnvLight> envLights;
    std::vector<float> envData;
    std::vector<DevInstance> instances;
    std::vector<float4> topEntry, topEntryWide;
    std::vector<float> lightFunc, lightCdf;
    float funcInt = 0.f, worldRadius = 0.f;
    float wbMin[3] = {0, 0, 0}, wbMax[3] = {0, 0, 0};
    int lightStrategy = 0;
    int voxN[3] = {1, 1, 1};
    uint32_t nPrims = 0;
    std::vector<uint32_t> topOrder;
    std::vector<std::vector<uint32_t>> objectOrder;
    std::vector<uint32_t> objectPrimBase;
    std::vector<int32_t> instanceObject;
    bool instanced = false, hasSubstrateBin = false;
    std::vector<uint8_t> primSingle;
    ShadowGrid shadowGrid;
};

int BuildSceneLayout(const HprtSceneDesc &d, SceneLayout *out);

void VoxelSamplePoints(float *out);

}
```

thesis-pbrt-v3_amd/csrc/shadow_grid.cpp:

```cpp
#include "shadow_grid.h"
#include <algorithm>
#include <chrono>
#include <cmath>
#include <cstdlib>
#include <cstring>

namespace hprt {

int ShadowGridModeFromEnv() { const char *e = getenv("HPRT_SHADOW_GRID"); return !e ? -1 : atoi(e) == 0 ? 0 : 1; }
uint32_t ShadowGridResFromEnv() {
    const char *e = getenv("HPRT_SHADOW_GRID_RES");
    const long v = e ? atol(e) : (long)SG_DEFAULT_RES;
    return (uint32_t)std::min(2048l, std::max(1l, v));
}

namespace {

struct D3 { double x, y, z; };
inline D3 operator-(D3 a, D3 b) { return {a.x - b.x, a.y - b.y, a.z - b.z}; }
inline D3 operator+(D3 a, D3 b) { return {a.x + b.x, a.y + b.y, a.z + b.z}; }
inline D3 operator*(D3 a, double s) { return {a.x * s, a.y * s, a.z * s}; }
inline double dot(D3 a, D3 b) { return a.x * b.x + a.y * b.y + a.z * b.z; }
inline D3 cross(D3 a, D3 b) { return {a.y * b.z - a.z * b.y, a.z * b.x - a.x * b.z, a.x * b.y - a.y * b.x}; }
inline double comp(D3 a, int k) { return k == 0 ? a.x : k == 1 ? a.y : a.z; }

double seg_dist2(D3 a, D3 b) {
    const D3 ab = b - a;
    const double l2 = dot(ab, ab);
    double t = l2 > 0 ? -dot(a, ab) / l2 : 0.0;
    t = std::min(1.0, std::max(0.0, t));
    const D3 p = a + ab * t;
    return dot(p, p);
}
double tri_dist2(D3 a, D3 b, D3 c) {
    double best = std::min(seg_dist2(a, b), std::min(seg_dist2(b, c), seg_dist2(c, a)));
    const D3 n = cross(b - a, c - a);
    const double n2 = dot(n, n);
    if (n2 > 0) {
        const double s = dot(a, n) / n2;
        const D3 q = n * s;
        const double e0 = dot(cross(b - a, q - a), n), e1 = dot(cross(c - b, q - b), n), e2 = dot(cross(a - c, q - c), n);
        if (e0 >= 0 && e1 >= 0 && e2 >= 0) best = std::min(best, dot(q, q));
    }
    return best;
}

bool face_rect(const D3 *poly, int n, int f, double lam, double r[4]) {
    const int ax = f >> 1; const double sg = (f & 1) ? -1.0 : 1.0;
    D3 out[8]; int no = 0;
    for (int i = 0; i < n; ++i) {
        const D3 p = poly[i], q = poly[(i + 1) % n];
        const double mp = sg * comp(p, ax) - lam, mq = sg * comp(q, ax) - lam;
        if (mp >= 0) out[no++] = p;
        if ((mp >= 0) != (mq >= 0)) { const double t = mp / (mp - mq); out[no++] = p + (q - p) * t; }
    }
    if (no == 0) return false;
    r[0] = r[2] = 1e300; r[1] = r[3] = -1e300;
    for (int i = 0; i < no; ++i) {
        const double m = std::max(sg * comp(out[i], ax), lam);
        const double u = comp(out[i], (ax + 1) % 3) / m, v = comp(out[i], (ax + 2) % 3) / m;
        r[0] = std::min(r[0], u); r[1] = std::max(r[1], u); r[2] = std::min(r[2], v); r[3] = std::max(r[3], v);
    }
    return true;
}

inline uint32_t f2u(float f) { uint32_t u; memcpy(&u, &f, 4); return u; }

}

void BuildShadowGrid(const float *tris, const uint8_t *single, uint32_t nPrims, const float light[3], const float bmin[3],
                     const float bmax[3], uint32_t R, size_t maxEntries, double maxCandidates, ShadowGrid *out) {
    const auto t0 = std::chrono::steady_clock::now();
    ShadowGrid &g = *out;
    g = ShadowGrid();
    for (int a = 0; a < 3; ++a) g.light[a] = light[a];
    double extent = 0;
    for (int a = 0; a < 3; ++a) extent = std::max(extent, (double)std::max(bmax[a], light[a]) - (double)std::min(bmin[a], light[a]));
    const double eps = SG_EPS_FACTOR * std::ldexp(1.0, -23) * extent;
    g.eps = eps;
    const D3 L = {light[0], light[1], light[2]};
    std::vector<SgEntry> nearList;
    struct Cover { uint32_t prim, key; double u0, u1, v0, v1; uint16_t face; };
    std::vector<Cover> covers;
    covers.reserve((size_t)nPrims * 2);
    for (uint32_t i = 0; i < nPrims; ++i) {
        const float *t = tris + 12 * (size_t)i;
        const D3 v[3] = {D3{t[0], t[1], t[2]} - L, D3{t[4], t[5], t[6]} - L, D3{t[8], t[9], t[10]} - L};
        const uint32_t word = i | ((single && single[i]) ? SG_SINGLE : 0u);
        const D3 n = cross(v[1] - v[0], v[2] - v[0]);
        const double d2 = tri_dist2(v[0], v[1], v[2]);
        const double D = std::sqrt(d2) - eps;
        const bool finite = std::isfinite(d2) && std::isfinite(dot(n, n));
        const double margin = D > 0 ? 4.0 * eps / D + std::ldexp(1.0, -20) : 1e300;
        if (!finite || dot(n, n) == 0 || !(D > 0) || margin > 0.5) { nearList.push_back({word, SG_RECT_ALL}); continue; }
        float kf = (float)(D * D);
        uint32_t kb = f2u(kf); kb = kb >= 2u ? kb - 2u : 0u;
        const double lam = D / 4;
        for (int f = 0; f < 6; ++f) {
            double r[4];
            if (!face_rect(v, 3, f, lam, r)) continue;
            r[0] -= margin; r[1] += margin; r[2] -= margin; r[3] += margin;
            if (r[1] < -1 || r[0] > 1 || r[3] < -1 || r[2] > 1) continue;
            covers.push_back({word, kb, r[0], r[1], r[2], r[3], (uint16_t)f});
        }
    }
    g.nNear = (uint32_t)nearList.size();
    if (maxCandidates > 0 && (double)nearList.size() > maxCandidates) { g = ShadowGrid(); return; }
    for (;; R = std::max(1u, R / 2)) {
        const double fineScale = 8.0 * R;
        auto fine = [&](double u) { const double c = std::floor((u + 1.0) * fineScale); return (uint32_t)std::min(16.0 * R - 1.0, std::max(0.0, c)); };
        const size_t nCells = (size_t)6 * R * R;
        std::vector<uint32_t> count(nCells + 1, 0u);
        size_t total = 0;
        bool over = false;
        for (const Cover &c : covers) {
            const uint32_t iu0 = fine(c.u0) >> 4, iu1 = fine(c.u1) >> 4, iv0 = fine(c.v0) >> 4, iv1 = fine(c.v1) >> 4;
            total += (size_t)(iu1 - iu0 + 1) * (iv1 - iv0 + 1);
            if (total > maxEntries) { over = true; break; }
            for (uint32_t iv = iv0; iv <= iv1; ++iv) for (uint32_t iu = iu0; iu <= iu1; ++iu) ++count[((size_t)c.face * R + iv) * R + iu];
        }
        if (over && R > 1) continue;
        if (over) { g = ShadowGrid(); return; }
        if (maxCandidates > 0 && (double)nearList.size() + (double)total / (double)nCells > maxCandidates) { g = ShadowGrid(); return; }
        g.R = R;
        g.cellStart.assign(nCells + 1, 0u);
        uint32_t at = g.nNear;
        for (size_t c = 0; c < nCells; ++c) { g.cellStart[c] = at; at += count[c]; g.longest = std::max(g.longest, count[c]); }
        g.cellStart[nCells] = at;
        g.entries.resize(at);
        std::copy(nearList.begin(), nearList.end(), g.entries.begin());
        std::vector<uint32_t> fill(g.cellStart.begin(), g.cellStart.end() - 1);
        for (const Cover &c : covers) {
            const uint32_t fu0 = fine(c.u0), fu1 = fine(c.u1), fv0 = fine(c.v0), fv1 = fine(c.v1);
            for (uint32_t iv = fv0 >> 4; iv <= fv1 >> 4; ++iv)
                for (uint32_t iu = fu0 >> 4; iu <= fu1 >> 4; ++iu) {
                    const uint32_t su0 = iu == fu0 >> 4 ? fu0 & 15u : 0u, su1 = iu == fu1 >> 4 ? fu1 & 15u : 15u;
                    const uint32_t sv0 = iv == fv0 >> 4 ? fv0 & 15u : 0u, sv1 = iv == fv1 >> 4 ? fv1 & 15u : 15u;
                    g.entries[fill[((size_t)c.face * R + iv) * R + iu]++] = {c.prim, (c.key & SG_KEY_MASK) | su0 | (su1 << 4) | (sv0 << 8) | (sv1 << 12)};
                }
        }
        for (size_t c = 0; c < nCells; ++c)
            std::sort(g.entries.begin() + g.cellStart[c], g.entries.begin() + g.cellStart[c + 1],
                      [](const SgEntry &a, const SgEntry &b) { return (a.key & SG_KEY_MASK) != (b.key & SG_KEY_MASK) ? (a.key & SG_KEY_MASK) < (b.key & SG_KEY_MASK) : (a.prim & SG_PRIM_MASK) < (b.prim & SG_PRIM_MASK); });
        break;
    }
    g.eligible = true;
    g.buildSeconds = std::chrono::duration<double>(std::chrono::steady_clock::now() - t0).count();
}

}
```

thesis-pbrt-v3_amd/csrc/shadow_grid.h:

```cpp
#pragma once
#include <cstddef>
#include <cstdint>
#include <vector>

namespace hprt {

enum : uint32_t { SG_SINGLE = 0x80000000u, SG_PRIM_MASK = 0x0fffffffu, SG_KEY_MASK = 0xffff0000u, SG_RECT_ALL = 0xf0f0u };
struct SgEntry { uint32_t prim, key; };
constexpr double SG_EPS_FACTOR = 128.0;
constexpr uint32_t SG_DEFAULT_RES = 512u;

struct ShadowGrid {
    bool eligible = false;
    uint32_t R = 0;
    float light[3] = {0, 0, 0};
    std::vector<uint32_t> cellStart;
    std::vector<SgEntry> entries;
    uint32_t nNear = 0, longest = 0;
    double eps = 0, buildSeconds = 0;
    size_t bytes() const { return cellStart.size() * sizeof(uint32_t) + entries.size() * sizeof(SgEntry); }
};

void BuildShadowGrid(const float *tris, const uint8_t *single, uint32_t nPrims, const float light[3], const float bmin[3],
                     const float bmax[3], uint32_t R, size_t maxEntries, double maxCandidates, ShadowGrid *out);

int ShadowGridModeFromEnv();
constexpr double SG_MAX_CANDIDATES = 14.0;
uint32_t ShadowGridResFromEnv();

}
```

Measured before the change: 6616 Mrays/s.

## Pack shadow grid into per-cell blocks with inline triangle vertices

Replaces the shadow grid's cellStart/entries index lists with a packed image. Each cell gets a 128-byte block holding its count, an overflow offset and the first two entries with their triangle vertices inlined. Longer lists continue as 48-byte records that carry the vertices and the next entry's key. The shadow-ray kernel's state machine is rewritten to read these blocks and records directly, removing the dependent loads of the cell header, the entry, and then the triangle. The cost is larger memory use from duplicated vertices, which may force a lower grid resolution under the byte cap, plus extra build-time packing.

```diff
diff --git a/thesis-pbrt-v3_amd/__init__.py b/thesis-pbrt-v3_amd/__init__.py
--- a/thesis-pbrt-v3_amd/__init__.py
+++ b/thesis-pbrt-v3_amd/__init__.py
@@ -357,6 +357,8 @@
     debug["hprt_debug_shadow_grid_info"] = (C.c_int, [vp, vp])
     debug["hprt_debug_shadow_grid_occluded"] = (C.c_int, [vp, sz, vp, vp, vp])
     debug["hprt_debug_shadow_grid_build"] = (C.c_int, [sz, vp, vp, C.c_uint32, vp, vp, sz, vp, sz])
+    debug["hprt_debug_shadow_grid_image"] = (C.c_int, [sz, vp, vp, C.c_uint32, vp, vp, sz, vp, sz])
+    debug["hprt_debug_shadow_grid_image_read"] = (C.c_int, [vp, vp, vp, sz, vp, sz])
     for name, (res, args) in list(sig.items()) + list(debug.items()):
         fn = getattr(lib, name)
         fn.restype = res
@@ -419,6 +421,49 @@
             "rect": np.stack([(entries[:, 1] >> s) & 15 for s in (0, 4, 8, 12)], axis=1).astype(np.int64)}
 
 
+SG_BLOCK_WORDS, SG_RECORD_WORDS, SG_BLOCK_SLOTS = 32, 12, 2
+
+
+def shadow_grid_image_decode(blocks, records, R, near):
+    blocks = np.asarray(blocks, np.uint32).reshape(6 * R * R, SG_BLOCK_WORDS)
+    records = np.asarray(records, np.uint32).reshape(-1, SG_RECORD_WORDS)
+    count = blocks[:, 0].astype(np.int64); overflow = blocks[:, 1].astype(np.int64)
+    cell_start = near + np.concatenate([[0], np.cumsum(count)])
+    n = int(cell_start[-1])
+    prim = np.zeros(n, np.uint32); key = np.zeros(n, np.uint32); nxt = np.zeros(n, np.uint32); verts = np.zeros((n, 9), np.uint32)
+    vcols = [0, 1, 2, 4, 5, 6, 8, 9, 10]
+
+    def from_records(dst, src):
+        prim[dst] = records[src, 3]; key[dst] = records[src, 7]; nxt[dst] = records[src, 11]; verts[dst] = records[src][:, vcols]
+
+    from_records(np.arange(near), np.arange(near))
+    for slot, (pw, kw, v0) in enumerate([((0, 2), (0, 3), 4), ((0, 7), (0, 11), 16)]):
+        cells = np.nonzero(count > slot)[0]
+        dst = cell_start[cells] + slot
+        prim[dst] = blocks[cells, pw[1]]; key[dst] = blocks[cells, kw[1]]
+        verts[dst] = blocks[cells][:, [v0 + c for c in vcols]]
+    over = np.maximum(count - SG_BLOCK_SLOTS, 0)
+    cells = np.repeat(np.arange(count.size), over)
+    k = np.arange(int(over.sum())) - np.repeat(np.cumsum(over) - over, over)
+    from_records(cell_start[cells] + SG_BLOCK_SLOTS + k, overflow[cells] + k)
+    return {"blocks": blocks, "records": records, "count": count, "overflow": overflow, "cell_start": cell_start, "prim_word": prim, "key_word": key,
+            "verts": verts, "next_key": nxt, "key2": blocks[:, 15]}
+
+
+def shadow_grid_image(p9, light, res):
+    p9 = np.ascontiguousarray(p9, np.float32).reshape(-1, 9)
+    light = np.ascontiguousarray(light, np.float32)
+    words = np.zeros(3, np.uint64)
+    _check(lib.hprt_debug_shadow_grid_image(p9.shape[0], _ptr(p9), _ptr(light), int(res), _ptr(words), None, 0, None, 0))
+    blocks = np.zeros(int(words[0]), np.uint32); records = np.zeros(int(words[1]), np.uint32)
+    _check(lib.hprt_debug_shadow_grid_image(p9.shape[0], _ptr(p9), _ptr(light), int(res), _ptr(words), _ptr(blocks), blocks.size, _ptr(records), records.size))
+    info = np.zeros(6, np.float64)
+    _check(lib.hprt_debug_shadow_grid_build(p9.shape[0], _ptr(p9), _ptr(light), int(res), _ptr(info), None, 0, None, 0))
+    out = shadow_grid_image_decode(blocks, records, int(res), int(info[2]))
+    out["words"] = tuple(int(w) for w in words)
+    return out
+
+
 def debug_halton_index(opt, px, py, sample):
     px = np.ascontiguousarray(px, np.int32); py = np.ascontiguousarray(py, np.int32); sample = np.ascontiguousarray(sample, np.int64)
     a = np.zeros(px.shape[0], np.uint64); b = np.zeros(px.shape[0], np.uint64); bounds = np.zeros(4, np.int32)
@@ -976,6 +1021,14 @@
         _check(lib.hprt_debug_shadow_grid_info(self._h, _ptr(out)))
         return {"eligible": bool(out[0]), "R": int(out[1]), "entries": int(out[2]), "near": int(out[3]), "bytes": int(out[4]), "build_seconds": float(out[5]),
                 "longest": int(out[6]), "mean": float(out[7]), "light": out[8:11].astype(np.float32), "render_launches": int(out[11])}
+
+    def shadow_grid_image(self):
+        words = np.zeros(2, np.uint64)
+        _check(lib.hprt_debug_shadow_grid_image_read(self._h, _ptr(words), None, 0, None, 0))
+        blocks = np.zeros(int(words[0]), np.uint32); records = np.zeros(max(1, int(words[1])), np.uint32)
+        _check(lib.hprt_debug_shadow_grid_image_read(self._h, _ptr(words), _ptr(blocks), blocks.size, _ptr(records), records.size))
+        info = self.shadow_grid_info()
+        return shadow_grid_image_decode(blocks, records[:int(words[1])], info["R"], info["near"])
 
     def shadow_grid_occluded_device(self, n, rays7_ptr, occ_ptr):
         ms = C.c_float()
diff --git a/thesis-pbrt-v3_amd/csrc/capi_device.hip b/thesis-pbrt-v3_amd/csrc/capi_device.hip
--- a/thesis-pbrt-v3_amd/csrc/capi_device.hip
+++ b/thesis-pbrt-v3_amd/csrc/capi_device.hip
@@ -167,12 +167,15 @@
     HIP_TRY(upload(sc->envLights, L.envLights)); HIP_TRY(upload(sc->envData, L.envData));
     if (L.shadowGrid.eligible) {
         const ShadowGrid &sg = L.shadowGrid;
-        static_assert(sizeof(SgEntry) == sizeof(uint2), "grid entries are read as 8-byte words");
-        std::vector<SgEntry> padded(sg.entries);
-        padded.push_back(SgEntry{0u, 0u});
-        HIP_TRY(upload(sc->sgCells, sg.cellStart)); HIP_TRY(upload(sc->sgEntries, padded));
-        sc->sg = DevShadowGrid{sc->sgCells.as<uint32_t>(), sc->sgEntries.as<uint2>(), (uint32_t)sg.entries.size(), sg.nNear, sg.R};
-        sc->sgInfo.longest = sg.longest; sc->sgInfo.buildSeconds = sg.buildSeconds; sc->sgInfo.eps = sg.eps; sc->sgInfo.bytes = sg.bytes();
+        const ShadowGridImage &im = L.shadowGridImage;
+        const size_t blockBytes = im.blocks.size() * sizeof(uint32_t), recordBytes = im.records.size() * sizeof(uint32_t);
+        if (blockBytes + recordBytes > 0xffff0000ull) return SetError(HPRT_E_INVALID, "hprt_scene_create: the shadow grid's image is too large");
+        HIP_TRY(sc->sgImage.alloc(blockBytes + recordBytes));
+        HIP_TRY(hipMemcpy(sc->sgImage.p, im.blocks.data(), blockBytes, hipMemcpyHostToDevice));
+        HIP_TRY(hipMemcpy((char *)sc->sgImage.p + blockBytes, im.records.data(), recordBytes, hipMemcpyHostToDevice));
+        sc->sg = DevShadowGrid{sc->sgImage.as<uint32_t>(), (uint32_t)(blockBytes + recordBytes), (uint32_t)blockBytes, sg.nNear, sg.R};
+        sc->sgInfo.nEntries = sg.entries.size(); sc->sgInfo.longest = sg.longest; sc->sgInfo.buildSeconds = sg.buildSeconds + im.packSeconds; sc->sgInfo.eps = sg.eps;
+        sc->sgInfo.bytes = im.bytes();
         for (int a = 0; a < 3; ++a) sc->sgInfo.light[a] = sg.light[a];
     }
     HIP_TRY(sc->counters.alloc(sizeof(DevCounters)));
@@ -310,22 +313,31 @@
 }
 static int g_shadowGrid = -1;
 static bool ShadowGridInUse(const HprtScene *s) {
-    return s->sg.entries != nullptr && g_shadowGrid != 0 && s->walk == HprtScene::Walk::Bvh && hprt::WideWalkInUse(s->dev) && !hprt::TraceProfileInUse();
+    return s->sg.image != nullptr && g_shadowGrid != 0 && s->walk == HprtScene::Walk::Bvh && hprt::WideWalkInUse(s->dev) && !hprt::TraceProfileInUse();
 }
 __attribute__((visibility("default"))) int hprt_debug_shadow_grid(int on) { const int was = g_shadowGrid; g_shadowGrid = on; return was; }
 __attribute__((visibility("default"))) int hprt_debug_shadow_grid_info(HprtScene *s, double out[12]) {
     if (!s || !out) return HPRT_E_INVALID;
     for (int a = 0; a < 3; ++a) out[8 + a] = s->sgInfo.light[a];
     out[11] = (double)s->sgInfo.renderLaunches;
-    const bool has = s->sg.entries != nullptr;
+    const bool has = s->sg.image != nullptr;
     const double nCells = has ? 6.0 * s->sg.R * s->sg.R : 1.0;
-    out[0] = has ? 1 : 0; out[1] = s->sg.R; out[2] = s->sg.nEntries; out[3] = s->sg.nNear; out[4] = (double)s->sgInfo.bytes;
-    out[5] = s->sgInfo.buildSeconds; out[6] = s->sgInfo.longest; out[7] = has ? (s->sg.nEntries - s->sg.nNear) / nCells : 0.0;
-    return HPRT_OK;
-}
+    out[0] = has ? 1 : 0; out[1] = s->sg.R; out[2] = (double)s->sgInfo.nEntries; out[3] = s->sg.nNear; out[4] = (double)s->sgInfo.bytes;
+    out[5] = s->sgInfo.buildSeconds; out[6] = s->sgInfo.longest; out[7] = has ? (double)(s->sgInfo.nEntries - s->sg.nNear) / nCells : 0.0;
+    return HPRT_OK;
+}
+__attribute__((visibility("default"))) int hprt_debug_shadow_grid_image_read(HprtScene *s, size_t words2[2], uint32_t *blocks, size_t block_cap, uint32_t *records, size_t record_cap) try {
+    if (!s || !words2) return SetError(HPRT_E_INVALID, "hprt_debug_shadow_grid_image_read: bad argument");
+    if (!s->sg.image) return SetError(HPRT_E_UNSUPPORTED, "hprt_debug_shadow_grid_image_read: the scene has no shadow grid");
+    HIP_TRY(hipSetDevice(s->device));
+    words2[0] = s->sg.recordsAt / sizeof(uint32_t); words2[1] = (s->sg.imageBytes - s->sg.recordsAt) / sizeof(uint32_t);
+    if (blocks && block_cap >= words2[0]) HIP_TRY(hipMemcpy(blocks, s->sg.image, words2[0] * sizeof(uint32_t), hipMemcpyDeviceToHost));
+    if (records && record_cap >= words2[1]) HIP_TRY(hipMemcpy(records, s->sg.image + words2[0], words2[1] * sizeof(uint32_t), hipMemcpyDeviceToHost));
+    return HPRT_OK;
+} catch (...) { return hprt::HandleException(); }
 __attribute__((visibility("default"))) int hprt_debug_shadow_grid_occluded(HprtScene *s, size_t n, const float *d_rays7, uint8_t *d_occ, float *ms) try {
     if (!s || !d_rays7 || !d_occ || n == 0 || n > 0x7ffffff0ull) return SetError(HPRT_E_INVALID, "hprt_debug_shadow_grid_occluded: bad argument");
-    if (!s->sg.entries) return SetError(HPRT_E_UNSUPPORTED, "hprt_debug_shadow_grid_occluded: the scene has no shadow grid");
+    if (!s->sg.image) return SetError(HPRT_E_UNSUPPORTED, "hprt_debug_shadow_grid_occluded: the scene has no shadow grid");
     HIP_TRY(hipSetDevice(s->device));
     SceneCall call(s, nullptr);
     RayStream rays; HitStream hits;
diff --git a/thesis-pbrt-v3_amd/csrc/capi_host.cpp b/thesis-pbrt-v3_amd/csrc/capi_host.cpp
--- a/thesis-pbrt-v3_amd/csrc/capi_host.cpp
+++ b/thesis-pbrt-v3_amd/csrc/capi_host.cpp
@@ -1834,4 +1834,29 @@
     return HPRT_OK;
 } catch (...) { return hprt::HandleException(); }
 
-}
+__attribute__((visibility("default"))) int hprt_debug_shadow_grid_image(size_t n, const float *p9, const float light[3], uint32_t R, size_t words3[3],
+                                                                         uint32_t *blocks, size_t block_cap, uint32_t *records, size_t record_cap) try {
+    if (!n || !p9 || !light || !words3 || R == 0 || n >= (1u << 28)) return SetError(HPRT_E_INVALID, "hprt_debug_shadow_grid_image: bad argument");
+    std::vector<float> tris(12 * n, 0.f);
+    std::vector<uint8_t> single(n, 1);
+    float lo[3] = {HPRT_INF, HPRT_INF, HPRT_INF}, hi[3] = {-HPRT_INF, -HPRT_INF, -HPRT_INF};
+    for (size_t i = 0; i < n; ++i)
+        for (int v = 0; v < 3; ++v)
+            for (int a = 0; a < 3; ++a) {
+                const float x = p9[9 * i + 3 * v + a];
+                tris[12 * i + 4 * v + a] = x;
+                if (x < lo[a]) lo[a] = x;
+                if (x > hi[a]) hi[a] = x;
+            }
+    ShadowGrid g;
+    BuildShadowGrid(tris.data(), single.data(), (uint32_t)n, light, lo, hi, R, (size_t)1 << 27, 0.0, &g);
+    if (!g.eligible || g.R != R) return SetError(HPRT_E_UNSUPPORTED, "hprt_debug_shadow_grid_image: the lists do not fit");
+    ShadowGridImage im;
+    PackShadowGrid(g, tris.data(), &im);
+    words3[0] = im.blocks.size(); words3[1] = im.records.size(); words3[2] = ShadowGridImageBytes(g) / sizeof(uint32_t);
+    if (blocks && block_cap >= im.blocks.size()) memcpy(blocks, im.blocks.data(), 4 * im.blocks.size());
+    if (records && record_cap >= im.records.size()) memcpy(records, im.records.data(), 4 * im.records.size());
+    return HPRT_OK;
+} catch (...) { return hprt::HandleException(); }
+
+}
diff --git a/thesis-pbrt-v3_amd/csrc/device/shadow_grid.h b/thesis-pbrt-v3_amd/csrc/device/shadow_grid.h
--- a/thesis-pbrt-v3_amd/csrc/device/shadow_grid.h
+++ b/thesis-pbrt-v3_amd/csrc/device/shadow_grid.h
@@ -3,7 +3,7 @@
 
 namespace hprt {
 
-struct DevShadowGrid { const uint32_t *cellStart; const uint2 *entries; uint32_t nEntries, nNear, R; };
+struct DevShadowGrid { const uint32_t *image; uint32_t imageBytes, recordsAt, nNear, R; };
 
 void LaunchShadowGrid(hipStream_t st, const DevScene &sc, const DevShadowGrid &g, const uint32_t *queue, const uint32_t *countPtr,
                       uint32_t countImm, uint32_t gridItems, const RayStream &rays, uint8_t *occ, uint32_t *workCounter);
diff --git a/thesis-pbrt-v3_amd/csrc/device/shadow_grid.hip b/thesis-pbrt-v3_amd/csrc/device/shadow_grid.hip
--- a/thesis-pbrt-v3_amd/csrc/device/shadow_grid.hip
+++ b/thesis-pbrt-v3_amd/csrc/device/shadow_grid.hip
@@ -32,23 +32,24 @@
     return su >= (w & 15u) && su <= ((w >> 4) & 15u) && sv >= ((w >> 8) & 15u) && sv <= ((w >> 12) & 15u);
 }
 
-enum : int { SG_IDLE = 0, SG_RAY = 1, SG_HEAD = 2, SG_FIRST = 3, SG_TEST = 4, SG_BOX = 5 };
+__device__ __forceinline__ float sg_key(uint32_t w) { return __uint_as_float(w & SG_KEY_MASK); }
+
+enum : int { SG_IDLE = 0, SG_RAY = 1, SG_BLOCK = 2, SG_BLOCK2 = 3, SG_OVER = 4, SG_BOX = 5 };
 
 __global__ __launch_bounds__(HPRT_TRACE_BLOCK, HPRT_SHADOW_GRID_WAVES)
 void k_shadow_grid(DevScene sc, DevShadowGrid g, const uint32_t *queue, const uint32_t *countPtr, uint32_t countImm, RayStream rays, uint8_t *occ,
                    uint32_t *workCounter, uint32_t chunk, uint32_t refillMin) {
     const uint32_t n = countPtr ? *countPtr : countImm;
     const uint32_t lane = __lane_id();
-    const auto triRsrc = __builtin_amdgcn_make_buffer_rsrc((void *)sc.tris, 0, (int)(sc.nPrims * 48u), 0x00020000);
     const auto boxRsrc = __builtin_amdgcn_make_buffer_rsrc((void *)sc.leafBox, 0, (int)(sc.nPrims * 32u), 0x00020000);
-    const auto entRsrc = __builtin_amdgcn_make_buffer_rsrc((void *)g.entries, 0, (int)((g.nEntries + 1u) * 8u), 0x00020000);
-    const auto cellRsrc = __builtin_amdgcn_make_buffer_rsrc((void *)g.cellStart, 0, (int)((6u * g.R * g.R + 1u) * 4u), 0x00020000);
+    const auto imgRsrc = __builtin_amdgcn_make_buffer_rsrc((void *)g.image, 0, (int)g.imageBytes, 0x00020000);
     const float robust = 1 + 2 * gamma_n(3);
     const float fineScale = 8.f * (float)g.R;
     int st = SG_IDLE;
     bool hit = false;
     uint32_t slot = 0u;
-    uint32_t i = 0u, end = 0u, i2 = 0u, end2 = 0u;
+    uint32_t i = 0u, cnt = 0u, recAt = 0u, kwN = 0u, cell = 0u;
+    bool nearList = false;
     uint32_t ePrim = 0u;
     uint32_t sub = 0u;
     vec3 ro, invDir;
@@ -91,32 +92,30 @@
         }
         u32x4 r0 = {0u, 0u, 0u, 0u}, r1 = {0u, 0u, 0u, 0u}, r2 = {0u, 0u, 0u, 0u};
         u32x4 r3 = {0u, 0u, 0u, 0u};
-        const uint32_t pi = ePrim & SG_PRIM_MASK;
-        if (st == SG_TEST) {
-            r0 = __builtin_amdgcn_raw_buffer_load_b128(triRsrc, pi * 48u, 0, 0);
-            r1 = __builtin_amdgcn_raw_buffer_load_b128(triRsrc, pi * 48u + 16u, 0, 0);
-            r2 = __builtin_amdgcn_raw_buffer_load_b128(triRsrc, pi * 48u + 32u, 0, 0);
-            if (i + 1u < end) r3 = __builtin_amdgcn_raw_buffer_load_b128(entRsrc, (i + 1u) * 8u, 0, 0);
-        } else if (st == SG_RAY) {
+        if (st == SG_RAY) {
             r0 = __builtin_bit_cast(u32x4, rays.a[slot]);
             r1 = __builtin_bit_cast(u32x4, rays.b[slot]);
-        } else if (st == SG_HEAD) {
-            const u32x2 h = __builtin_amdgcn_raw_buffer_load_b64(cellRsrc, i * 4u, 0, 0);
-            r3.x = h.x; r3.y = h.y;
-        } else if (st == SG_FIRST) {
-            r3 = __builtin_amdgcn_raw_buffer_load_b128(entRsrc, i * 8u, 0, 0);
         } else if (st == SG_BOX) {
+            const uint32_t pi = ePrim & SG_PRIM_MASK;
             r0 = __builtin_amdgcn_raw_buffer_load_b128(boxRsrc, pi * 32u, 0, 0);
             r1 = __builtin_amdgcn_raw_buffer_load_b128(boxRsrc, pi * 32u + 16u, 0, 0);
+        } else if (st != SG_IDLE) {
+            const uint32_t at = st == SG_BLOCK ? cell * 128u + 16u : st == SG_BLOCK2 ? cell * 128u + 64u : recAt;
+            r0 = __builtin_amdgcn_raw_buffer_load_b128(imgRsrc, at, 0, 0);
+            r1 = __builtin_amdgcn_raw_buffer_load_b128(imgRsrc, at + 16u, 0, 0);
+            r2 = __builtin_amdgcn_raw_buffer_load_b128(imgRsrc, at + 32u, 0, 0);
+            if (st == SG_BLOCK) r3 = __builtin_amdgcn_raw_buffer_load_b128(imgRsrc, cell * 128u, 0, 0);
         }
         asm volatile("" : "+v"(r0), "+v"(r1), "+v"(r2), "+v"(r3));
         auto leaf_reached = [&](float lx, float ly, float lz, float hx, float hy, float hz) -> bool {
             float tEn;
             return slab_test(lx, hx, ly, hy, lz, hz, ro, invDir, invDir.x < 0, invDir.y < 0, invDir.z < 0, robust, &tEn) && tEn < rayTMax;
         };
+        const int st0 = st;
         bool done = false;
-        bool haveNext = false;
-        if (st == SG_RAY) {
+        bool listEnd = false;
+        bool doTest = false;
+        if (st0 == SG_RAY) {
             ro = vec3(__uint_as_float(r0.x), __uint_as_float(r0.y), __uint_as_float(r0.z));
             rayTMax = __uint_as_float(r0.w);
             const vec3 d(__uint_as_float(r1.x), __uint_as_float(r1.y), __uint_as_float(r1.z));
@@ -124,40 +123,62 @@
             shear = ray_shear(d, invDir);
             const float dist2 = d.x * d.x + d.y * d.y + d.z * d.z;
             lim = rayTMax <= 1.f ? dist2 * (1.f + 0x1p-20f) : HPRT_INF;
-            i = sg_cell(d, g.R, fineScale, &sub);
-            st = SG_HEAD;
-        } else if (st == SG_HEAD) {
-            if (g.nNear != 0u) { i = 0u; end = g.nNear; i2 = r3.x; end2 = r3.y; }
-            else { i = r3.x; end = r3.y; i2 = end2 = 0u; }
-            st = SG_FIRST;
-            if (i >= end) done = true;
-        } else if (st == SG_FIRST) {
-            haveNext = true;
-        } else if (st == SG_TEST) {
+            cell = sg_cell(d, g.R, fineScale, &sub);
+            i = 0u;
+            if (g.nNear != 0u) { nearList = true; cnt = g.nNear; recAt = g.recordsAt; st = SG_OVER; }
+            else { nearList = false; st = SG_BLOCK; }
+        } else if (st0 == SG_BLOCK) {
+            cnt = r3.x; recAt = g.recordsAt + r3.y * 48u;
+            if (i == 0u) {
+                if (cnt == 0u || sg_key(r3.w) > lim) listEnd = true;
+                else if (sg_reaches(r3.w, sub)) { doTest = true; ePrim = r3.z; }
+            }
+        } else if (st0 == SG_BLOCK2) {
+            doTest = true;
+        } else if (st0 == SG_OVER) {
+            if (sg_key(r1.w) > lim) listEnd = true;
+            else if (sg_reaches(r1.w, sub)) { doTest = true; ePrim = r0.w; }
+        } else if (st0 == SG_BOX) {
+            if (leaf_reached(__uint_as_float(r0.x), __uint_as_float(r0.y), __uint_as_float(r0.z), __uint_as_float(r0.w), __uint_as_float(r1.x), __uint_as_float(r1.y))) { hit = true; done = true; }
+            else {
+                ++i;
+                if (nearList || i > 2u) recAt += 48u;
+                if (!nearList && i < 2u) st = SG_BLOCK;
+                else if (i >= cnt) listEnd = true;
+                else st = SG_OVER;
+            }
+        }
+        bool boxWanted = false;
+        if (doTest) {
             asm volatile("" : "+v"(r0), "+v"(r1), "+v"(r2));
             const vec3 p0(__uint_as_float(r0.x), __uint_as_float(r0.y), __uint_as_float(r0.z)), p1(__uint_as_float(r1.x), __uint_as_float(r1.y), __uint_as_float(r1.z)),
                        p2(__uint_as_float(r2.x), __uint_as_float(r2.y), __uint_as_float(r2.z));
             float b0, b1, b2, t;
-            bool boxWanted = false;
             if (tri_test(p0, p1, p2, ro, rayTMax, shear, &b0, &b1, &b2, &t)) {
                 if (ePrim & SG_SINGLE) {
                     if (leaf_reached(fminf(fminf(p0.x, p1.x), p2.x), fminf(fminf(p0.y, p1.y), p2.y), fminf(fminf(p0.z, p1.z), p2.z),
                                      fmaxf(fmaxf(p0.x, p1.x), p2.x), fmaxf(fmaxf(p0.y, p1.y), p2.y), fmaxf(fmaxf(p0.z, p1.z), p2.z))) { hit = true; done = true; }
                 } else boxWanted = true;
             }
-            if (boxWanted) st = SG_BOX;
-            else if (!done) { ++i; haveNext = true; }
-        } else if (st == SG_BOX) {
-            if (leaf_reached(__uint_as_float(r0.x), __uint_as_float(r0.y), __uint_as_float(r0.z), __uint_as_float(r0.w), __uint_as_float(r1.x), __uint_as_float(r1.y))) { hit = true; done = true; }
-            else { ++i; st = SG_FIRST; if (i >= end) { i = i2; end = end2; i2 = end2 = 0u; if (i >= end) done = true; } }
-        }
-        if (haveNext) {
-            const bool in0 = i < end && !(__uint_as_float(r3.y & SG_KEY_MASK) > lim);
-            const bool in1 = in0 && i + 1u < end && !(__uint_as_float(r3.w & SG_KEY_MASK) > lim);
-            if (in0 && sg_reaches(r3.y, sub)) { ePrim = r3.x; st = SG_TEST; }
-            else if (in1 && sg_reaches(r3.w, sub)) { ePrim = r3.z; ++i; st = SG_TEST; }
-            else if (in1) { i += 2u; st = SG_FIRST; if (i >= end) { i = i2; end = end2; i2 = end2 = 0u; if (i >= end) done = true; } }
-            else { i = i2; end = end2; i2 = end2 = 0u; st = SG_FIRST; if (i >= end) done = true; }
+        }
+        if (boxWanted) st = SG_BOX;
+        else if (!done && !listEnd) {
+            if (st0 == SG_BLOCK) {
+                i = 1u;
+                if (cnt <= 1u || sg_key(r1.w) > lim) listEnd = true;
+                else if (sg_reaches(r1.w, sub)) { st = SG_BLOCK2; ePrim = r0.w; kwN = r2.w; }
+                else { i = 2u; if (cnt <= 2u || sg_key(r2.w) > lim) listEnd = true; else st = SG_OVER; }
+            } else if (st0 == SG_BLOCK2) {
+                i = 2u;
+                if (cnt <= 2u || sg_key(kwN) > lim) listEnd = true; else st = SG_OVER;
+            } else if (st0 == SG_OVER) {
+                ++i; recAt += 48u;
+                if (i >= cnt || sg_key(r2.w) > lim) listEnd = true;
+            }
+        }
+        if (listEnd) {
+            if (nearList) { nearList = false; i = 0u; st = SG_BLOCK; }
+            else done = true;
         }
         if (done) { occ[slot] = hit ? 1 : 0; st = SG_IDLE; }
     }
diff --git a/thesis-pbrt-v3_amd/csrc/device_state.h b/thesis-pbrt-v3_amd/csrc/device_state.h
--- a/thesis-pbrt-v3_amd/csrc/device_state.h
+++ b/thesis-pbrt-v3_amd/csrc/device_state.h
@@ -65,8 +65,8 @@
     hprt::DevBuf nodes, tris, primVtx, primN, vUV, vS, shapes, materials, lights, spheres, instances, topEntry, topEntryWide, lightFunc, lightCdf, perms, primes, primeSums, primeMagic;
     hprt::DevBuf envLights, envData;
     hprt::DevBuf wide, leafBox;
-    hprt::DevBuf sgCells, sgEntries; hprt::DevShadowGrid sg{};
-    struct ShadowGridInfo { uint32_t longest = 0; double buildSeconds = 0, eps = 0; size_t bytes = 0; float light[3] = {0, 0, 0}; uint64_t renderLaunches = 0; } sgInfo;
+    hprt::DevBuf sgImage; hprt::DevShadowGrid sg{};
+    struct ShadowGridInfo { size_t nEntries = 0; uint32_t longest = 0; double buildSeconds = 0, eps = 0; size_t bytes = 0; float light[3] = {0, 0, 0}; uint64_t renderLaunches = 0; } sgInfo;
     hprt::DevBuf counters, workCounter, deepStack;
     struct Capture { int bounce = -1, kind = 0; float *out7 = nullptr; size_t cap = 0, n = 0; } capture;
     bool shadeCountsOn = false; uint64_t shadeDeferred = 0, shadeRetried = 0;
diff --git a/thesis-pbrt-v3_amd/csrc/scene_layout.cpp b/thesis-pbrt-v3_amd/csrc/scene_layout.cpp
--- a/thesis-pbrt-v3_amd/csrc/scene_layout.cpp
+++ b/thesis-pbrt-v3_amd/csrc/scene_layout.cpp
@@ -535,7 +535,16 @@
     for (uint32_t i = 0; i < L.nPrims; ++i) if ((f2u(L.tris[3 * (size_t)i].w) & TAG_KIND_MASK) != 0u) return HPRT_OK;
     static_assert(sizeof(float4) == 16, "triangle records are read as 12 floats per primitive");
     const size_t capMb = [] { const char *e = getenv("HPRT_SHADOW_GRID_MAX_MB"); return e ? (size_t)std::max(1l, atol(e)) : (size_t)1024; }();
-    BuildShadowGrid(&L.tris[0].x, L.primSingle.data(), L.nPrims, L.lights[0].pos, L.wbMin, L.wbMax, ShadowGridResFromEnv(), capMb * ((1u << 20) / sizeof(SgEntry)), mode < 0 ? SG_MAX_CANDIDATES : 0.0, &L.shadowGrid);
+    const size_t capBytes = std::min(capMb << 20, (size_t)0xffff0000u);
+    for (uint32_t R = ShadowGridResFromEnv();; R = std::max(1u, L.shadowGrid.R / 2)) {
+        while (R > 1 && (size_t)6 * R * R * SG_BLOCK_WORDS * sizeof(uint32_t) > capBytes) R /= 2;
+        const size_t maxEntries = capBytes / (SG_RECORD_WORDS * sizeof(uint32_t)) + (size_t)SG_BLOCK_SLOTS * 6 * R * R;
+        BuildShadowGrid(&L.tris[0].x, L.primSingle.data(), L.nPrims, L.lights[0].pos, L.wbMin, L.wbMax, R, maxEntries, mode < 0 ? SG_MAX_CANDIDATES : 0.0, &L.shadowGrid);
+        if (!L.shadowGrid.eligible) return HPRT_OK;
+        if (ShadowGridImageBytes(L.shadowGrid) <= capBytes) break;
+        if (L.shadowGrid.R == 1) { L.shadowGrid = ShadowGrid(); return HPRT_OK; }
+    }
+    PackShadowGrid(L.shadowGrid, &L.tris[0].x, &L.shadowGridImage);
     return HPRT_OK;
 }
 
diff --git a/thesis-pbrt-v3_amd/csrc/scene_layout.h b/thesis-pbrt-v3_amd/csrc/scene_layout.h
--- a/thesis-pbrt-v3_amd/csrc/scene_layout.h
+++ b/thesis-pbrt-v3_amd/csrc/scene_layout.h
@@ -37,6 +37,7 @@
     bool instanced = false, hasSubstrateBin = false;
     std::vector<uint8_t> primSingle;
     ShadowGrid shadowGrid;
+    ShadowGridImage shadowGridImage;
 };
 
 int BuildSceneLayout(const HprtSceneDesc &d, SceneLayout *out);
diff --git a/thesis-pbrt-v3_amd/csrc/shadow_grid.cpp b/thesis-pbrt-v3_amd/csrc/shadow_grid.cpp
--- a/thesis-pbrt-v3_amd/csrc/shadow_grid.cpp
+++ b/thesis-pbrt-v3_amd/csrc/shadow_grid.cpp
@@ -148,4 +148,51 @@
     g.buildSeconds = std::chrono::duration<double>(std::chrono::steady_clock::now() - t0).count();
 }
 
+size_t ShadowGridImageBytes(const ShadowGrid &g) {
+    const size_t nCells = g.cellStart.empty() ? 0 : g.cellStart.size() - 1;
+    size_t nRecords = g.nNear;
+    for (size_t c = 0; c < nCells; ++c) {
+        const uint32_t n = g.cellStart[c + 1] - g.cellStart[c];
+        if (n > SG_BLOCK_SLOTS) nRecords += n - SG_BLOCK_SLOTS;
+    }
+    return (nCells * SG_BLOCK_WORDS + (nRecords + SG_PAD_RECORDS) * SG_RECORD_WORDS) * sizeof(uint32_t);
 }
+
+void PackShadowGrid(const ShadowGrid &g, const float *tris, ShadowGridImage *out) {
+    const auto t0 = std::chrono::steady_clock::now();
+    ShadowGridImage &im = *out;
+    im = ShadowGridImage();
+    im.R = g.R; im.nNear = g.nNear;
+    const size_t nCells = (size_t)6 * g.R * g.R;
+    im.nRecords =(ShadowGridImageBytes(g) / sizeof(uint32_t) - nCells * SG_BLOCK_WORDS) / SG_RECORD_WORDS - SG_PAD_RECORDS;
+    im.blocks.assign(nCells * SG_BLOCK_WORDS, 0u);
+    im.records.assign((im.nRecords + SG_PAD_RECORDS) * SG_RECORD_WORDS, 0u);
+    auto put = [&](uint32_t *w, const SgEntry &e, int vertex, uint32_t fourth) {
+        memcpy(w, tris + 12 * (size_t)(e.prim & SG_PRIM_MASK) + 4 * vertex, 12);
+        w[3] = fourth;
+    };
+    auto run = [&](size_t at, uint32_t a, uint32_t b) {
+        for (uint32_t k = a; k < b; ++k, ++at) {
+            uint32_t *w = im.records.data() + at * SG_RECORD_WORDS;
+            const SgEntry &e = g.entries[k];
+            put(w, e, 0, e.prim); put(w + 4, e, 1, e.key); put(w + 8, e, 2, k + 1 < b ? g.entries[k + 1].key : 0u);
+        }
+        return at;
+    };
+    size_t at = run(0, 0u, g.nNear);
+    for (size_t c = 0; c < nCells; ++c) {
+        const uint32_t a = g.cellStart[c], n = g.cellStart[c + 1] - a;
+        uint32_t *w = im.blocks.data() + c * SG_BLOCK_WORDS;
+        const SgEntry *e = g.entries.data() + a;
+        w[0] = n; w[1] = (uint32_t)at;
+        if (n > 0) {
+            w[2] = e[0].prim; w[3] = e[0].key;
+            put(w + 4, e[0], 0, n > 1 ? e[1].prim : 0u); put(w + 8, e[0], 1, n > 1 ? e[1].key : 0u); put(w + 12, e[0], 2, n > 2 ? e[2].key : 0u);
+        }
+        if (n > 1) { put(w + 16, e[1], 0, 0u); put(w + 20, e[1], 1, 0u); put(w + 24, e[1], 2, 0u); }
+        if (n > SG_BLOCK_SLOTS) at = run(at, a + SG_BLOCK_SLOTS, a + n);
+    }
+    im.packSeconds = std::chrono::duration<double>(std::chrono::steady_clock::now() - t0).count();
+}
+
+}
diff --git a/thesis-pbrt-v3_amd/csrc/shadow_grid.h b/thesis-pbrt-v3_amd/csrc/shadow_grid.h
--- a/thesis-pbrt-v3_amd/csrc/shadow_grid.h
+++ b/thesis-pbrt-v3_amd/csrc/shadow_grid.h
@@ -24,6 +24,18 @@
 void BuildShadowGrid(const float *tris, const uint8_t *single, uint32_t nPrims, const float light[3], const float bmin[3],
                      const float bmax[3], uint32_t R, size_t maxEntries, double maxCandidates, ShadowGrid *out);
 
+enum : uint32_t { SG_BLOCK_WORDS = 32u, SG_BLOCK_SLOTS = 2u, SG_RECORD_WORDS = 12u, SG_PAD_RECORDS = 1u };
+struct ShadowGridImage {
+    uint32_t R = 0, nNear = 0;
+    size_t nRecords = 0;
+    std::vector<uint32_t> blocks;
+    std::vector<uint32_t> records;
+    double packSeconds = 0;
+    size_t bytes() const { return (blocks.size() + records.size()) * sizeof(uint32_t); }
+};
+size_t ShadowGridImageBytes(const ShadowGrid &g);
+void PackShadowGrid(const ShadowGrid &g, const float *tris, ShadowGridImage *out);
+
 int ShadowGridModeFromEnv();
 constexpr double SG_MAX_CANDIDATES = 14.0;
 uint32_t ShadowGridResFromEnv();
```

Result: faster. 7060 Mrays/s, median of 6 (+6.7%).
